# madmann91/bvh

Measured on AMD Instinct MI355X. Metric: Mrays/s closest-hit (1M-tri scene), higher is better.
Workload: dtype f32; 1 GPU; soup_1m: 1,000,000-triangle random soup (M3), worst-case incoherent; robust traversal, DefaultBuilder with thread pool (mini-trees) Quality::High built on the GPU (the reference's default configuration is thread pool + High); rays reordered for coherence inside the timed pass (library default for this tree size); tris=1000000, nodes=1866439, ray_batches=4, parallelism=single GPU, launched_by=single process

## Files before the change

bvh_amd/_lib.py:

```python
from __future__ import annotations

import ctypes as C
import os

HERE = os.path.dirname(os.path.abspath(__file__))
LIB_PATH = os.environ.get("BVH_AMD_LIB") or os.path.join(HERE, "lib", "libbvh_amd.so")

_lib = None


class BvhAmdError(RuntimeError):
    pass


class BuildConfig(C.Structure):
    _fields_ = [("quality", C.c_int), ("min_leaf_size", C.c_size_t), ("max_leaf_size", C.c_size_t),
                ("parallel_threshold", C.c_size_t)]


class Counters(C.Structure):
    _fields_ = [("node_pairs", C.c_ulonglong), ("prim_tests", C.c_ulonglong), ("leaves", C.c_ulonglong)]


class MiniTreeConfig(C.Structure):
# ... 37 lines not shown
    "bvh_amd_probe_record_walk": (_I, [_P, C.c_uint32, C.c_uint32, _I, _I, C.POINTER(C.c_float), C.POINTER(C.c_ulonglong), _P]),
    "bvh_amd_probe_mixed_walk": (_I, [_P, C.c_uint32, _P, C.c_uint32, C.c_uint32, _I, _I, _I, C.POINTER(C.c_float), C.POINTER(C.c_ulonglong), _P]),
    "bvh_amd_probe_record_walk_ex": (_I, [_P, C.c_uint32, C.c_uint32, _I, _I, _I, _I, C.POINTER(C.c_float), C.POINTER(C.c_ulonglong), _P]),
    "bvh_amd_release_cached_memory": (_I, []),
    "bvh_amd_cached_scratch_bytes": (_Z, []),
    "bvh_amd_scratch_cache_limit": (_Z, []),
    "bvh_amd_device_count": (_I, []),
    "bvh_amd_device_name": (_I, [_I, C.c_char_p, _Z]),
    "bvh_amd_device_select": (_I, [_I]),
    "bvh_amd_device_current": (_I, []),
    "bvh_amd_comm_unique_id": (_I, [_P]),
    "bvh_amd_comm_create": (_P, [_P, _I, _I]),
    "bvh_amd_comm_adopt": (_P, [_P]),
    "bvh_amd_comm_destroy": (None, [_P]),
    "bvh_amd_comm_rank": (_I, [_P]),
    "bvh_amd_comm_size": (_I, [_P]),
    "bvh_amd_comm_handle": (_P, [_P]),
    "bvh_amd_comm_broadcast": (_I, [_P, _P, _Z, _I, _P]),
    "bvh_amd_comm_cache_clear": (_I, []),
    "bvh_amd_rccl_library": (C.c_char_p, []),
    "bvh_thread_pool_create": (_P, [_Z]),
    "bvh_thread_pool_destroy": (None, [_P]),
    "bvh_amd_gather": (_I, [_P, _P, _Z, _Z, _P, _P]),
    "bvh_amd_pinhole_rays3f": (_I, [_P, _P, _P, _Z, _Z, _P, _P]),
    "bvh_amd_pinhole_rays3d": (_I, [_P, _P, _P, _Z, _Z, _P, _P]),
    "bvh_amd_shade_eyelight3f": (_I, [_P, _P, _P, _Z, _P, _P]),
    "bvh_amd_shade_eyelight3d": (_I, [_P, _P, _P, _Z, _P, _P]),
    "bvh_amd_device_alloc": (_P, [_Z]),
    "bvh_amd_device_free": (None, [_P]),
    "bvh_amd_copy_to_device": (_I, [_P, _P, _Z]),
    "bvh_amd_copy_to_host": (_I, [_P, _P, _Z]),
    "bvh_amd_synchronize": (_I, [_P]),
    "bvh_amd_std_sort_ids3f": (_I, [_P, _Z, _P, _P]),
    "bvh_amd_std_sort_ids3d": (_I, [_P, _Z, _P, _P]),
    "bvh_amd_radix_sort_pairs_u32": (_I, [_P, _P, _Z, _I, _P]),
}
_SIGS_T = {
    "bvh{S}_build": (_P, [_P, _P, _P, _Z, _P]),
    "bvh{S}_build_device": (_P, [_P, _P, _Z, _P, _I, _P]),
    "bvh{S}_build_sah": (_P, [_P, _P, _P, _Z, _P, _P]),
    "bvh{S}_build_device_sah": (_P, [_P, _P, _Z, _P, _I, _P, _P]),
    "bvh{S}_build_device_binned": (_P, [_P, _P, _Z, _P, _P, _Z, _P]),
    "bvh{S}_build_minitree_device": (_P, [_P, _P, _Z, _P, _P]),
    "bvh{S}_from_nodes": (_P, [_P, _Z, _P, _Z]),
    "bvh{S}_extract": (_P, [_P, _Z]),
    "bvh{S}_destroy": (None, [_P]),
    "bvh{S}_optimize": (None, [_P, _P]),
    "bvh{S}_optimize_config": (_I, [_P, _P]),
    "bvh{S}_refit": (None, [_P]),
    "bvh{S}_refit_status": (_I, [_P]),
    "bvh{S}_sync_device": (_I, [_P]),
    "bvh{S}_refit_boxes": (_I, [_P, _P, _Z, _P]),
    "bvh{S}_refit_tris": (_I, [_P, _P, _Z, _P, _P]),
    "bvh{S}_traversal_cost": (_I, [_P, C.POINTER(C.c_double), _P]),
    "bvh{S}_append_node": (None, [_P]),
    "bvh{S}_remove_last_node": (None, [_P]),
    "bvh_node{S}_set_prim_count": (None, [_P, _Z]),
    "bvh_node{S}_set_first_id": (None, [_P, _Z]),
    "bvh_node{S}_set_bbox": (None, [_P, _P]),
    "bvh{S}_save": (None, [_P, _P]),
    "bvh{S}_load": (_P, [_P]),
    "bvh{S}_serialize": (_Z, [_P, _P, _Z]),
    "bvh{S}_deserialize": (_P, [_P, _Z]),
    "bvh{S}_serialize_device": (_Z, [_P, _P, _Z, _P]),
    "bvh{S}_deserialize_device": (_P, [_P, _Z, _P]),
    "bvh{S}_broadcast": (_P, [_P, _I, _P, _P, _Z, C.POINTER(C.c_void_p), C.POINTER(C.c_size_t), _P]),
    "bvh{S}_replicate": (_I, [_P, _P, _Z, _I, C.POINTER(C.c_int), C.POINTER(C.c_void_p), C.POINTER(C.c_void_p)]),
    "bvh{S}_get_node": (_P, [_P, _Z]),
    "bvh{S}_get_prim_id": (_Z, [_P, _Z]),
    "bvh{S}_get_prim_count": (_Z, [_P]),
    "bvh{S}_get_node_count": (_Z, [_P]),
    "bvh_node{S}_is_leaf": (C.c_bool, [_P]),
    "bvh_node{S}_get_prim_count": (_Z, [_P]),
    "bvh_node{S}_get_first_id": (_Z, [_P]),
    "bvh{S}_copy_nodes": (None, [_P, _P]),
    "bvh{S}_copy_prim_ids": (None, [_P, _P]),
    "bvh{S}_device_prim_ids": (_P, [_P]),
    "bvh_amd_tri_bounds{S}": (_I, [_P, _Z, _P, _P, _P]),
    "bvh_amd_precompute_tris{S}": (_I, [_P, _P, _Z, _P, _P]),
    "bvh_amd_sphere_bounds{S}": (_I, [_P, _Z, _P, _P, _P]),
    "bvh{S}_intersect_rays_tri": (_I, [_P, _P, _P, _Z, _U, _P, _P, _P]),
    "bvh{S}_intersect_rays_sphere": (_I, [_P, _P, _P, _Z, _U, _P, _P, _P]),
    "bvh{S}_prepare_trace": (_I, [_P, _Z, _P]),
    "bvh{S}_closest_points_tri": (_I, [_P, _P, _P, _Z, _U, _P, _P, _P]),
    "bvh{S}_closest_points_sphere": (_I, [_P, _P, _P, _Z, _U, _P, _P, _P]),
    "bvh{S}_intersect_ray": (None, [_P, _P, _P]),
    "bvh{S}_intersect_ray_any": (None, [_P, _P, _P]),
    "bvh{S}_intersect_ray_robust": (None, [_P, _P, _P]),
    "bvh{S}_intersect_ray_any_robust": (None, [_P, _P, _P]),
    "bvh{S}_intersect_ray_visit": (_I, [_P, _P, _Z, _U, _P]),
}


class OptimizeProfile(C.Structure):
    _fields_ = [("iterations", C.c_uint), ("replayed", C.c_uint), ("replacements", C.c_ulonglong), ("heap_ms", C.c_float)]


class SahConfig(C.Structure):
    _fields_ = [("log_cluster_size", C.c_size_t), ("cost_ratio", C.c_double)]


class OptimizeConfig(C.Structure):
    _fields_ = [("batch_size_ratio", C.c_double), ("max_iter_count", C.c_size_t)]


def ray_visitor_types(suffix: str):
    scalar = C.c_float if suffix[1] == "f" else C.c_double
    leaf_t = C.CFUNCTYPE(C.c_bool, C.c_void_p, C.POINTER(scalar), C.c_size_t, C.c_size_t)
    inner_t = C.CFUNCTYPE(None, C.c_void_p, C.c_size_t)

    class Visitor(C.Structure):
        _fields_ = [("user_data", C.c_void_p), ("leaf_fn", leaf_t), ("inner_fn", inner_t)]
    return Visitor, leaf_t, inner_t


_ONLY_3D = ("bvh_amd_tri_bounds{S}", "bvh_amd_precompute_tris{S}", "bvh{S}_intersect_rays_tri", "bvh{S}_prepare_trace",
            "bvh{S}_build_minitree_device",
            "bvh{S}_closest_points_tri", "bvh{S}_closest_points_sphere",
            "bvh{S}_refit_tris", "bvh{S}_traversal_cost")


def exported_symbols():
    names = list(_SIGS)
    for s in ("3f", "3d", "2f", "2d"):
        names += [k.format(S=s) for k in _SIGS_T if s[0] == "3" or k not in _ONLY_3D]
        names += [f"bvh_node{s}_get_bbox"]
    return names


def load():
    global _lib
    if _lib is not None:
        return _lib
    import torch
    if not os.path.exists(LIB_PATH):
        raise BvhAmdError(f"{LIB_PATH} is missing: build it with `python -m bvh_amd.build` "
                          "(no fallback path exists)")
    lib = C.CDLL(LIB_PATH)
    for name, (res, args) in _SIGS.items():
        f = getattr(lib, name)
        f.restype, f.argtypes = res, args
    for s in ("3f", "3d", "2f", "2d"):
        for name, (res, args) in _SIGS_T.items():
            if s[0] == "2" and name in _ONLY_3D:
                continue
            f = getattr(lib, name.format(S=s))
            f.restype, f.argtypes = res, args
    lib.bvh_node3f_get_bbox.restype, lib.bvh_node3f_get_bbox.argtypes = BBox3f, [_P]
    lib.bvh_node3d_get_bbox.restype, lib.bvh_node3d_get_bbox.argtypes = BBox3d, [_P]
    lib.bvh_node2f_get_bbox.restype, lib.bvh_node2f_get_bbox.argtypes = BBox2f, [_P]
    lib.bvh_node2d_get_bbox.restype, lib.bvh_node2d_get_bbox.argtypes = BBox2d, [_P]
    _lib = lib
    return lib


def last_error() -> str:
    return load().bvh_amd_last_error().decode()


def check(rc: int, what: str):
    if rc != 0:
        raise BvhAmdError(f"{what} failed ({rc}): {last_error()}")
```

bvh_amd/api.py:

```python
from __future__ import annotations

import ctypes as C
import enum
from dataclasses import dataclass, field

import numpy as np

from . import _lib

INVALID = 0xFFFFFFFF
HITF = np.dtype([("prim", "<u4"), ("t", "<f4"), ("u", "<f4"), ("v", "<f4")])
HITD = np.dtype([("prim", "<u4"), ("pad", "<u4"), ("t", "<f8"), ("u", "<f8"), ("v", "<f8")])
NODEF = np.dtype([("bounds", "<f4", (6,)), ("index", "<u4")])
NODED = np.dtype([("bounds", "<f8", (6,)), ("index", "<u8")])
NODE2F = np.dtype([("bounds", "<f4", (4,)), ("index", "<u4")])
NODE2D = np.dtype([("bounds", "<f8", (4,)), ("index", "<u8")])
_NODE_DTYPES = {"3f": NODEF, "3d": NODED, "2f": NODE2F, "2d": NODE2D}


class Quality(enum.IntEnum):
    Low = 0
    Medium = 1
    High = 2

# ... 94 lines not shown
        return np.float32 if self._s[1] == "f" else np.float64

    @property
    def dim(self) -> int:
        return int(self._s[0])

    @property
    def node_count(self) -> int:
        return self._f("bvh{S}_get_node_count")(self._h)

    @property
    def prim_count(self) -> int:
        return self._f("bvh{S}_get_prim_count")(self._h)

    @property
    def nodes(self) -> np.ndarray:
        out = np.empty(self.node_count, dtype=_NODE_DTYPES[self._s])
        self._f("bvh{S}_copy_nodes")(self._h, out.ctypes.data_as(C.c_void_p))
        return out

    @property
    def prim_ids(self) -> np.ndarray:
        out = np.empty(self.prim_count, dtype=np.uint64)
        self._f("bvh{S}_copy_prim_ids")(self._h, out.ctypes.data_as(C.c_void_p))
        return out

    def device_prim_ids(self):
        torch = _torch()
        ptr = self._f("bvh{S}_device_prim_ids")(self._h)
        n = self.prim_count

        class _Holder:
            __cuda_array_interface__ = {"shape": (n,), "typestr": "<i4", "data": (ptr, False), "version": 2}
        t = torch.as_tensor(_Holder(), device="cuda")
        t._bvh_keepalive = self
        return t

    def optimize(self, thread_pool=None, batch_size_ratio=None, max_iter_count=None):
        _torch()
        if batch_size_ratio is not None or max_iter_count is not None:
            cfg = _lib.OptimizeConfig(0.05 if batch_size_ratio is None else float(batch_size_ratio),
                                      3 if max_iter_count is None else int(max_iter_count))
            _lib.check(self._f("bvh{S}_optimize_config")(self._h, C.byref(cfg)), "optimize")
            return
        _lib.check(self._f("bvh{S}_optimize_config")(self._h, None), "optimize")

    def refit(self):
        _torch()
        _lib.check(self._f("bvh{S}_refit_status")(self._h), "refit")

    def _prims_in(self, x, cols, what):
        torch = _torch()
        if not hasattr(x, "dtype"):
            x = np.asarray(x)
        dt = x.dtype
        want = torch.float32 if self._s[1] == "f" else torch.float64
        if dt not in (want, np.dtype(self.dtype), self.dtype):
            raise TypeError(f"{what}: the tree is {np.dtype(self.dtype).name}, the array is {dt}")
        return _dev(x, cols)

    def refit_boxes(self, bboxes):
        bb = self._prims_in(bboxes, 2 * self.dim, "refit_boxes")
        _lib.check(self._f("bvh{S}_refit_boxes")(self._h, bb.data_ptr(), bb.shape[0], _stream()), "refit_boxes")

    def refit_tris(self, tris9, out=None):
        torch = _torch()
        if self.dim != 3:
            raise TypeError("refit_tris: triangles are 3D (tri.h)")
        t = self._prims_in(tris9, 9, "refit_tris")
        if out is None:
            out = torch.empty((self.prim_count, 12), dtype=t.dtype, device=t.device)
        elif not (isinstance(out, torch.Tensor) and out.is_cuda and out.is_contiguous() and out.dtype == t.dtype and out.numel() == 12 * self.prim_count):
            raise TypeError("refit_tris: `out` must be a contiguous (prim_count, 12) device tensor of the tree's scalar type")
        _lib.check(self._f("bvh{S}_refit_tris")(self._h, t.data_ptr(), t.shape[0], out.data_ptr(), _stream()), "refit_tris")
        return out.reshape(-1, 12)

    def traversal_cost(self) -> float:
        _torch()
        if self.dim != 3:
            raise TypeError("traversal_cost: 3D trees only")
        cost = C.c_double(0.0)
        _lib.check(self._f("bvh{S}_traversal_cost")(self._h, C.byref(cost), _stream()), "traversal_cost")
        return float(cost.value)

    def set_node_bbox(self, node_id: int, lo, hi):
        node = self._f("bvh{S}_get_node")(self._h, node_id)
        ct = C.c_float if self._s[1] == "f" else C.c_double
        bb = (ct * (2 * self.dim))(*[float(v) for v in list(lo) + list(hi)])
        self._f("bvh_node{S}_set_bbox")(node, bb)

    def sync_device(self):
        _lib.check(self._f("bvh{S}_sync_device")(self._h), "sync_device")

    def sync_host(self):
        if not self._f("bvh{S}_get_node")(self._h, 0):
            raise _lib.BvhAmdError(_lib.last_error())

    def get_root(self):
        return self.nodes[0]

    def serialize(self) -> bytes:
        n = self._f("bvh{S}_serialize")(self._h, None, 0)
        buf = C.create_string_buffer(n)
        self._f("bvh{S}_serialize")(self._h, buf, n)
        return buf.raw

    @staticmethod
    def deserialize(data: bytes, dtype=np.float32, dim: int = 3) -> "Bvh":
        s = _suffix(np.dtype(dtype), dim)
        lib = _lib.load()
        _torch()
        return Bvh(getattr(lib, f"bvh{s}_deserialize")(data, len(data)), s)

    def serialize_device(self):
        torch = _torch()
        n = self._f("bvh{S}_serialize_device")(self._h, None, 0, _stream())
        buf = torch.empty(n, dtype=torch.uint8, device="cuda")
        if self._f("bvh{S}_serialize_device")(self._h, buf.data_ptr(), n, _stream()) != n:
            raise _lib.BvhAmdError(_lib.last_error())
        return buf

    @staticmethod
    def deserialize_device(buf, dtype=np.float32, dim: int = 3) -> "Bvh":
        torch = _torch()
        s = _suffix(np.dtype(dtype), dim)
        if not (buf.is_cuda and buf.dtype == torch.uint8 and buf.is_contiguous()):
            raise TypeError("deserialize_device takes a contiguous uint8 tensor resident on the GPU")
        return Bvh(getattr(_lib.load(), f"bvh{s}_deserialize_device")(buf.data_ptr(), buf.numel(), _stream()), s)

    def intersect_ray(self, ray, leaf_fn, any_hit: bool = False, robust: bool = False, inner_fn=None, start=None):
        lib = _lib.load()
        dt = np.float32 if self._s[1] == "f" else np.float64
        r = np.ascontiguousarray(ray, dtype=dt).reshape(2 * self.dim + 2)
        Visitor, leaf_t, inner_t = _lib.ray_visitor_types(self._s)
        failure = []

        def on_leaf(_user, t, begin, end):
            try:
                hit, new_t = leaf_fn(dt(t[0]), int(begin), int(end))
                t[0] = new_t
                return bool(hit)
            except BaseException as exc:
                failure.append(exc)
                t[0] = float("-inf")
                return True

        def on_inner(_user, first):
            try:
                if not failure:
                    inner_fn(int(first))
            except BaseException as exc:
                failure.append(exc)

        v = Visitor(None, leaf_t(on_leaf), inner_t(on_inner) if inner_fn is not None else inner_t())
        if start is None:
            start = (1 << 64) - 1
        rc = getattr(lib, f"bvh{self._s}_intersect_ray_visit")(self._h, r.ctypes.data, int(start), (RayFlags.ANY_HIT if any_hit else 0) | (RayFlags.ROBUST if robust else 0), C.byref(v))
        if failure:
            raise failure[0]
        _lib.check(rc, "intersect_ray_visit")

    def extract_bvh(self, root_id: int) -> "Bvh":
        h = getattr(_lib.load(), f"bvh{self._s}_extract")(self._h, int(root_id))
        return Bvh(h, self._s)

    @staticmethod
# ... 250 lines not shown
```

bvh_amd/csrc/capi.hip:

```cpp
#include "common.h"

#include <cstring>
#include <memory>

namespace bvh_amd {

template <typename T> int reinsertion_optimize_device(HostNode<T>* d_nodes, size_t node_count, hipStream_t stream, int dim);
template <typename T>
int reinsertion_optimize_config_device(HostNode<T>* d_nodes, size_t node_count, hipStream_t stream, int dim, double batch_size_ratio, size_t iterations);
void reinsertion_stats(unsigned out[2]);
void last_optimize_profile(bvh_amd_optimize_profile* out);
template <typename T>
int build_minitree_explicit(BvhImpl<T>& out, const T* d_bboxes, const T* d_centers, size_t n, const bvh_build_config& cfg, bool prune, T ratio,
                            bool optimize, uint32_t log2_grid, hipStream_t stream);
template <typename T>
int extract_device(BvhImpl<T>& out, const HostNode<T>* d_nodes, size_t node_count, const uint32_t* d_ids, size_t root_id, hipStream_t stream);
template <typename T> int refit_device(HostNode<T>* d_nodes, size_t node_count, hipStream_t stream);
template <typename T> int reachable_node_count(const HostNode<T>* d_nodes, size_t node_count, hipStream_t stream, size_t* out);
template <typename T> int relayout_on_device(BvhImpl<T>& b, const HostNode<T>* d_nodes, hipStream_t stream);

namespace {
thread_local std::string g_error;
}

// ... 221 lines not shown
    if (rc) return rc;
    rc = relayout_on_device<T>(b, b.d_nodes, nullptr);
    if (rc) return rc;
    HostNode<T> root;
    BVH_HIP_TRY(hipMemcpy(&root, b.d_nodes, sizeof(root), hipMemcpyDeviceToHost), BVH_AMD_ERR_HIP);
    b.root_index = static_cast<uint32_t>(root.index);
    for (int k = 0; k < 6; ++k) b.root_bounds[k] = root.bounds[k];
    if (b.host_valid) BVH_HIP_TRY(hipMemcpy(b.nodes.data(), b.d_nodes, bytes, hipMemcpyDeviceToHost), BVH_AMD_ERR_HIP);
    b.nodes2_valid = false;
    return BVH_AMD_OK;
}

template <typename T> BvhImpl<T>* extract(BvhImpl<T>* pb, size_t root_id) {
    if (!pb) { set_error("extract: null bvh"); return nullptr; }
    BvhImpl<T>& b = *pb;
    if (make_nodes_resident<T>(b)) return nullptr;
    if (!b.d_prim_ids) { set_error("extract: the BVH has no device prim ids"); return nullptr; }
    auto out = std::make_unique<BvhImpl<T>>();
    out->dim = b.dim;
    if (extract_device<T>(*out, b.d_nodes, b.node_count, b.d_prim_ids, root_id, nullptr)) return nullptr;
    return out.release();
}

template <typename T> int whole_array_is_one_tree(const HostNode<T>* d, size_t n) {
    size_t reachable = 0;
    const int rc = reachable_node_count<T>(d, n, nullptr, &reachable);
    if (rc) return rc;
    if (reachable != n)
        return fail(BVH_AMD_ERR_UNSUPPORTED, "optimize: " + std::to_string(n - reachable) + " of the " + std::to_string(n) +
                    " nodes are not reachable from the root (unused sibling pairs); extract_bvh(0) first, or remove them");
    return BVH_AMD_OK;
}
template <typename T> int optimize(BvhImpl<T>* b) {
    const int dim = b ? b->dim : 3;
    return on_resident_nodes<T>(b, [dim](HostNode<T>* d, size_t n) {
        const int rc = whole_array_is_one_tree<T>(d, n);
        return rc ? rc : reinsertion_optimize_device<T>(d, n, nullptr, dim);
    });
}
template <typename T> int optimize_config(BvhImpl<T>* b, const bvh_amd_optimize_config* config) {
    const int dim = b ? b->dim : 3;
    const bvh_amd_optimize_config c = config ? *config : bvh_amd_optimize_config{0.05, 3};
    return on_resident_nodes<T>(b, [dim, c](HostNode<T>* d, size_t n) {
        const int rc = whole_array_is_one_tree<T>(d, n);
        return rc ? rc : reinsertion_optimize_config_device<T>(d, n, nullptr, dim, c.batch_size_ratio, c.max_iter_count);
    });
}
template <typename T> int refit(BvhImpl<T>* b) {
    return on_resident_nodes<T>(b, [](HostNode<T>* d, size_t n) { return refit_device<T>(d, n, nullptr); });
}

template <typename T>
int refit_prims(BvhImpl<T>* pb, int src_kind, const T* d_src, size_t n_src, T* d_tris12_out, void* stream_, const char* who) {
    if (!pb) return fail(BVH_AMD_ERR_ARG, std::string(who) + ": null bvh");
    if (!d_src) return fail(BVH_AMD_ERR_ARG, std::string(who) + ": null primitive array");
    BvhImpl<T>& b = *pb;
    hipStream_t stream = static_cast<hipStream_t>(stream_);
    int cur = -1;
    BVH_HIP_TRY(hipGetDevice(&cur), BVH_AMD_ERR_HIP);
    if (cur != b.device) return fail(BVH_AMD_ERR_ARG, std::string(who) + ": BVH lives on another device than the current one");
    if (b.node_count == 0 || !b.d_prim_ids) return fail(BVH_AMD_ERR_ARG, std::string(who) + ": BVH has no device copy");
    if (b.max_prim_id < 0) {
        uint32_t largest = 0;
        const int rc = max_prim_id_device(b.d_prim_ids, b.prim_count, stream, &largest);
        if (rc) return rc;
        b.max_prim_id = largest;
    }
    if (b.prim_count && n_src <= static_cast<size_t>(b.max_prim_id))
        return fail(BVH_AMD_ERR_ARG, std::string(who) + ": " + std::to_string(n_src) + " primitives given, but prim_ids refers to primitive " +
                    std::to_string(b.max_prim_id) + " (the array is indexed by original primitive id)");
    const bool from_host = b.host_valid || !b.d_nodes || b.d_nodes_count != b.node_count;
    int rc = from_host ? b.wait_refit() : BVH_AMD_OK;
    if (rc) return rc;
    rc = make_nodes_resident<T>(b);
    if (rc) return rc;
    if (from_host || (b.pair_count && !b.d_pairs)) {
        const long long largest = b.max_prim_id;
        rc = relayout_on_device<T>(b, b.d_nodes, stream);
        if (rc) return rc;
        b.max_prim_id = largest;
    }
    rc = refit_prims_device<T>(b.d_nodes, b.d_pairs, b.node_count, src_kind, d_src, n_src, b.d_prim_ids, b.prim_count, stream);
    if (rc == BVH_AMD_OK && d_tris12_out) rc = launch_precompute_tris<T>(d_src, b.d_prim_ids, b.prim_count, d_tris12_out, stream);
    b.host_valid = false;
    b.nodes2_valid = false;
    const int rc2 = b.note_refit(stream);
    return rc ? rc : rc2;
}

template <typename T>
int traversal_cost_checked(const BvhImpl<T>* b, double* cost_out, void* stream) {
    if (!b || !cost_out) return fail(BVH_AMD_ERR_ARG, "traversal_cost: null bvh or output");
    int cur = -1;
    BVH_HIP_TRY(hipGetDevice(&cur), BVH_AMD_ERR_HIP);
    if (cur != b->device) return fail(BVH_AMD_ERR_ARG, "traversal_cost: BVH lives on another device than the current one");
    return traversal_cost<T>(*b, cost_out, static_cast<hipStream_t>(stream));
}

template <typename T> int sync_device(BvhImpl<T>* pb) {
    if (!pb) return fail(BVH_AMD_ERR_ARG, "sync_device: null bvh");
    BvhImpl<T>& b = *pb;
    int rc = b.dim == 2 ? b.sync_host2() : b.sync_host();
    if (rc) return rc;
    if (b.dim == 2) b.widen_host();
    if (b.d_nodes) { (void)hipFree(b.d_nodes); b.d_nodes = nullptr; }
    return upload_bvh<T>(b, nullptr);
}

template <typename T> struct CTypes2;
template <> struct CTypes2<float>  { using Bvh = bvh2f; using Node = bvh_node2f; using BBox = bvh_bbox2f; using Vec = bvh_vec2f; using Ray = bvh_ray2f; };
template <> struct CTypes2<double> { using Bvh = bvh2d; using Node = bvh_node2d; using BBox = bvh_bbox2d; using Vec = bvh_vec2d; using Ray = bvh_ray2d; };
template <typename T> BvhImpl<T>* impl2(typename CTypes2<T>::Bvh* b) { return reinterpret_cast<BvhImpl<T>*>(b); }
template <typename T> const BvhImpl<T>* impl2(const typename CTypes2<T>::Bvh* b) { return reinterpret_cast<const BvhImpl<T>*>(b); }
template <typename T> typename CTypes2<T>::Bvh* handle2(BvhImpl<T>* b) { return reinterpret_cast<typename CTypes2<T>::Bvh*>(b); }

template <typename T>
typename CTypes2<T>::Bvh* build2_device(const T* d_bb4, const T* d_cc2, size_t n, const bvh_build_config* config, bvh_amd_builder builder, void* stream) {
    if (!d_bb4 || !d_cc2 || n == 0) { set_error("build: empty input (the reference's behaviour is undefined for 0 primitives)"); return nullptr; }
    bvh_build_config cfg = config ? *config : default_config();
    if (cfg.min_leaf_size < 1 || cfg.min_leaf_size > cfg.max_leaf_size || cfg.max_leaf_size > 15) {
        set_error("build: need 1 <= min_leaf_size <= max_leaf_size <= 15 (4-bit primitive count, index.h:38)");
        return nullptr;
    }
    T *d_bb6 = nullptr, *d_cc3 = nullptr;
    BVH_HIP_TRY_PTR(hipMalloc(&d_bb6, n * 6 * sizeof(T)));
    hipError_t e = hipMalloc(&d_cc3, n * 3 * sizeof(T));
    auto b = std::make_unique<BvhImpl<T>>();
    b->dim = 2;
    int rc = e == hipSuccess ? launch_widen_inputs<T>(d_bb4, d_cc2, n, d_bb6, d_cc3, static_cast<hipStream_t>(stream))
                             : fail(BVH_AMD_ERR_HIP, std::string("build: ") + hipGetErrorString(e));
    if (rc == BVH_AMD_OK) rc = build_on_device<T>(*b, d_bb6, d_cc3, n, cfg, builder, static_cast<hipStream_t>(stream));
    (void)hipStreamSynchronize(static_cast<hipStream_t>(stream));
    (void)hipFree(d_bb6);
    if (d_cc3) (void)hipFree(d_cc3);
    return rc == BVH_AMD_OK ? handle2<T>(b.release()) : nullptr;
}

template <typename T>
typename CTypes2<T>::Bvh* build2_host(bvh_thread_pool* pool, const typename CTypes2<T>::BBox* bboxes, const typename CTypes2<T>::Vec* centers, size_t n,
                                      const bvh_build_config* config) {
    if (!bboxes || !centers || n == 0) { set_error("build: empty input"); return nullptr; }
    static_assert(sizeof(typename CTypes2<T>::BBox) == 4 * sizeof(T) && sizeof(typename CTypes2<T>::Vec) == 2 * sizeof(T));
    T *d_bb = nullptr, *d_cc = nullptr;
    BVH_HIP_TRY_PTR(hipMalloc(&d_bb, n * 4 * sizeof(T)));
    hipError_t e = hipMalloc(&d_cc, n * 2 * sizeof(T));
    if (e == hipSuccess) e = hipMemcpy(d_bb, bboxes, n * 4 * sizeof(T), hipMemcpyHostToDevice);
    if (e == hipSuccess) e = hipMemcpy(d_cc, centers, n * 2 * sizeof(T), hipMemcpyHostToDevice);
    typename CTypes2<T>::Bvh* out = nullptr;
    if (e == hipSuccess)
        out = build2_device<T>(d_bb, d_cc, n, config, pool ? BVH_AMD_BUILDER_DEFAULT_PARALLEL : BVH_AMD_BUILDER_DEFAULT_SERIAL, nullptr);
    else
        set_error(std::string("build: ") + hipGetErrorString(e));
    (void)hipDeviceSynchronize();
    (void)hipFree(d_bb);
    if (d_cc) (void)hipFree(d_cc);
    return out;
}

template <typename T>
BvhImpl<T>* adopt_nodes2(const HostNode2<T>* nodes, size_t nn, std::vector<size_t>&& ids) {
    auto b = std::make_unique<BvhImpl<T>>();
    b->dim = 2;
    b->nodes2.assign(nodes, nodes + nn);
    b->widen_host();
    b->prim_ids = std::move(ids);
    if (upload_bvh<T>(*b, nullptr) != BVH_AMD_OK) return nullptr;
// ... 234 lines not shown
        return build_minitree<T>(d_bb, d_cc, n, cfg, stream); }                                                     \
    bvh##S* bvh##S##_extract(bvh##S* b, size_t root_id) { return handle<T>(extract<T>(impl<T>(b), root_id)); }      \
    bvh##S* bvh##S##_from_nodes(const void* nodes, size_t nn, const size_t* ids, size_t np) {                       \
        return from_nodes<T>(nodes, nn, ids, np); }                                                                 \
    void bvh##S##_destroy(bvh##S* b) { delete impl<T>(b); }                                                         \
    void bvh##S##_optimize(bvh_thread_pool*, bvh##S* b) { loud_or_abort(optimize<T>(impl<T>(b)), "bvh" #S "_optimize"); } \
    int bvh##S##_optimize_config(bvh##S* b, const bvh_amd_optimize_config* c) { return optimize_config<T>(impl<T>(b), c); } \
    void bvh##S##_refit(bvh##S* b) { loud_or_abort(refit<T>(impl<T>(b)), "bvh" #S "_refit"); }                     \
    int bvh##S##_refit_status(bvh##S* b) { return refit<T>(impl<T>(b)); }                                           \
    int bvh##S##_sync_device(bvh##S* b) { return sync_device<T>(impl<T>(b)); }                                       \
    int bvh##S##_refit_boxes(bvh##S* b, const T* d_bb, size_t n, void* s) {                                         \
        return refit_prims<T>(impl<T>(b), REFIT_BOXES3, d_bb, n, nullptr, s, "refit_boxes"); }                       \
    int bvh##S##_refit_tris(bvh##S* b, const T* d_tris9, size_t n, T* d_tris12_out, void* s) {                      \
        return refit_prims<T>(impl<T>(b), REFIT_TRIS, d_tris9, n, d_tris12_out, s, "refit_tris"); }                  \
    int bvh##S##_traversal_cost(bvh##S* b, double* cost_out, void* s) { return traversal_cost_checked<T>(impl<T>(b), cost_out, s); } \
    void bvh##S##_append_node(bvh##S* b) {                                                                          \
        if (impl<T>(b)->sync_host() != BVH_AMD_OK) return;                                                           \
        impl<T>(b)->nodes.emplace_back(); impl<T>(b)->node_count = impl<T>(b)->nodes.size(); }                       \
    void bvh##S##_remove_last_node(bvh##S* b) {                                                                     \
        if (impl<T>(b)->sync_host() != BVH_AMD_OK || impl<T>(b)->nodes.empty()) return;                              \
        impl<T>(b)->nodes.pop_back(); impl<T>(b)->node_count = impl<T>(b)->nodes.size(); }                           \
    void bvh_node##S##_set_prim_count(bvh_node##S* n, size_t c) {                                                   \
        auto h = reinterpret_cast<HostNode<T>*>(n);                                                                 \
        h->index = (h->index & ~static_cast<IndexOf<T>::Type>(kCountMask)) | (static_cast<IndexOf<T>::Type>(c) & kCountMask); } \
    void bvh_node##S##_set_first_id(bvh_node##S* n, size_t f) {                                                     \
        auto h = reinterpret_cast<HostNode<T>*>(n);                                                                 \
        h->index = (static_cast<IndexOf<T>::Type>(f) << kCountBits) | (h->index & kCountMask); }                    \
    void bvh_node##S##_set_bbox(bvh_node##S* n, const bvh_bbox##S* bb) {                                            \
        auto h = reinterpret_cast<HostNode<T>*>(n);                                                                 \
        h->bounds[0] = bb->min.x; h->bounds[1] = bb->max.x; h->bounds[2] = bb->min.y; h->bounds[3] = bb->max.y;     \
        h->bounds[4] = bb->min.z; h->bounds[5] = bb->max.z; }                                                         \
    void bvh##S##_save(const bvh##S* b, FILE* f) { if (b && f) save<T>(*impl<T>(b), f); }                           \
    bvh##S* bvh##S##_load(FILE* f) { return f ? load<T>(f) : nullptr; }                                             \
    size_t bvh##S##_serialize(const bvh##S* b, void* out, size_t cap) { return b ? serialize<T>(*impl<T>(b), out, cap) : 0; } \
    bvh##S* bvh##S##_deserialize(const void* bytes, size_t size) { return deserialize<T>(bytes, size); }            \
    size_t bvh##S##_serialize_device(bvh##S* b, void* d_out, size_t cap, void* stream) { return serialize_device<T>(impl<T>(b), d_out, cap, stream); } \
    bvh##S* bvh##S##_deserialize_device(const void* d_bytes, size_t size, void* stream) {                           \
        return handle<T>(deserialize_from_device<T>(d_bytes, size, 3, static_cast<hipStream_t>(stream))); }         \
    bvh_node##S* bvh##S##_get_node(bvh##S* b, size_t i) {                                                          \
        if (impl<T>(b)->sync_host() != BVH_AMD_OK) return nullptr;                                                   \
        return reinterpret_cast<bvh_node##S*>(&impl<T>(b)->nodes[i]); }                                              \
    size_t bvh##S##_get_prim_id(const bvh##S* b, size_t i) {                                                        \
        if (impl<T>(b)->sync_host() != BVH_AMD_OK) return BVH_INVALID_PRIM_ID;                                       \
        return impl<T>(b)->prim_ids[i]; }                                                                            \
    size_t bvh##S##_get_prim_count(const bvh##S* b) { return impl<T>(b)->prim_count; }                              \
    size_t bvh##S##_get_node_count(const bvh##S* b) { return impl<T>(b)->node_count; }                              \
    bool bvh_node##S##_is_leaf(const bvh_node##S* n) { return (reinterpret_cast<const HostNode<T>*>(n)->index & kCountMask) != 0; } \
    size_t bvh_node##S##_get_prim_count(const bvh_node##S* n) { return reinterpret_cast<const HostNode<T>*>(n)->index & kCountMask; } \
    size_t bvh_node##S##_get_first_id(const bvh_node##S* n) { return reinterpret_cast<const HostNode<T>*>(n)->index >> kCountBits; } \
    bvh_bbox##S bvh_node##S##_get_bbox(const bvh_node##S* n) {                                                      \
        auto h = reinterpret_cast<const HostNode<T>*>(n);                                                           \
        bvh_bbox##S r; r.min.x = h->bounds[0]; r.max.x = h->bounds[1]; r.min.y = h->bounds[2]; r.max.y = h->bounds[3]; \
        r.min.z = h->bounds[4]; r.max.z = h->bounds[5]; return r; }                                                 \
    void bvh##S##_copy_nodes(const bvh##S* b, void* out) {                                                          \
        if (impl<T>(b)->sync_host() != BVH_AMD_OK) return;                                                           \
        std::memcpy(out, impl<T>(b)->nodes.data(), impl<T>(b)->nodes.size() * sizeof(HostNode<T>)); }               \
    void bvh##S##_copy_prim_ids(const bvh##S* b, size_t* out) {                                                     \
        if (impl<T>(b)->sync_host() != BVH_AMD_OK) return;                                                           \
        std::memcpy(out, impl<T>(b)->prim_ids.data(), impl<T>(b)->prim_ids.size() * sizeof(size_t)); }              \
    const uint32_t* bvh##S##_device_prim_ids(const bvh##S* b) { return impl<T>(b)->d_prim_ids; }                    \
    int bvh_amd_tri_bounds##S(const T* t, size_t n, T* bb, T* cc, void* s) {                                        \
        return launch_tri_bounds<T>(t, n, bb, cc, static_cast<hipStream_t>(s)); }                                   \
    int bvh_amd_precompute_tris##S(const T* t, const uint32_t* perm, size_t n, T* out, void* s) {                   \
        return launch_precompute_tris<T>(t, perm, n, out, static_cast<hipStream_t>(s)); }                           \
    int bvh_amd_sphere_bounds##S(const T* sp, size_t n, T* bb, T* cc, void* s) {                                    \
        return launch_sphere_bounds<T>(sp, n, bb, cc, static_cast<hipStream_t>(s)); }                               \
    int bvh##S##_intersect_rays_tri(const bvh##S* b, const T* prims, const bvh_ray##S* rays, size_t n, unsigned flags, \
                                    bvh_hit##S* hits, bvh_amd_counters* cnt, void* s) {                             \
        return intersect<T>(b, LEAF_TRIANGLE, prims, rays, n, flags, hits, cnt, s); }                               \
    int bvh##S##_intersect_rays_sphere(const bvh##S* b, const T* prims, const bvh_ray##S* rays, size_t n, unsigned flags, \
                                       bvh_hit##S* hits, bvh_amd_counters* cnt, void* s) {                          \
        return intersect<T>(b, LEAF_SPHERE, prims, rays, n, flags, hits, cnt, s); }                                 \
    int bvh##S##_closest_points_tri(const bvh##S* b, const T* prims, const T* queries, size_t n, unsigned flags,       \
                                    bvh_hit##S* hits, bvh_amd_counters* cnt, void* s) {                             \
        return closest<T>(b, LEAF_TRIANGLE, prims, queries, n, flags, hits, cnt, s); }                              \
    int bvh##S##_closest_points_sphere(const bvh##S* b, const T* prims, const T* queries, size_t n, unsigned flags,    \
                                       bvh_hit##S* hits, bvh_amd_counters* cnt, void* s) {                          \
        return closest<T>(b, LEAF_SPHERE, prims, queries, n, flags, hits, cnt, s); }                                \
    int bvh##S##_prepare_trace(const bvh##S* b, size_t n_rays_hint, void* s) {                                      \
        if (!b) return fail(BVH_AMD_ERR_ARG, "prepare_trace: null bvh");                                            \
        int cur = -1;                                                                                               \
        BVH_HIP_TRY(hipGetDevice(&cur), BVH_AMD_ERR_HIP);                                                           \
        if (cur != impl<T>(b)->device) return fail(BVH_AMD_ERR_ARG, "prepare_trace: BVH lives on another device than the current one"); \
        return prepare_trace<T>(*impl<T>(b), n_rays_hint, static_cast<hipStream_t>(s)); }

BVH_AMD_IMPL(float, 3f)
BVH_AMD_IMPL(double, 3d)

#define BVH_AMD_IMPL_RAY(T, S, CB, VIS, D, IMPL)                                                                         \
    void bvh##S##_intersect_ray(const bvh##S* b, const bvh_ray##S* r, const CB* cb) { intersect_ray_legacy<T, D>(IMPL<T>(b), r, cb, 0u); } \
    void bvh##S##_intersect_ray_any(const bvh##S* b, const bvh_ray##S* r, const CB* cb) {                           \
        intersect_ray_legacy<T, D>(IMPL<T>(b), r, cb, BVH_AMD_RAY_ANY_HIT); }                                        \
    void bvh##S##_intersect_ray_robust(const bvh##S* b, const bvh_ray##S* r, const CB* cb) {                        \
        intersect_ray_legacy<T, D>(IMPL<T>(b), r, cb, BVH_AMD_RAY_ROBUST); }                                         \
    void bvh##S##_intersect_ray_any_robust(const bvh##S* b, const bvh_ray##S* r, const CB* cb) {                    \
        intersect_ray_legacy<T, D>(IMPL<T>(b), r, cb, BVH_AMD_RAY_ANY_HIT | BVH_AMD_RAY_ROBUST); }                   \
    int bvh##S##_intersect_ray_visit(const bvh##S* b, const bvh_ray##S* r, size_t start, unsigned flags, const VIS* v) { \
        if (!v || !v->leaf_fn) return fail(BVH_AMD_ERR_ARG, "intersect_ray_visit: null visitor");                   \
        return intersect_ray_visit<T, D>(IMPL<T>(b), r, start, flags, v->leaf_fn, v->inner_fn, v->user_data); }

BVH_AMD_IMPL_RAY(float, 3f, bvh_intersect_callbackf, bvh_amd_ray_visitorf, 3, impl)
BVH_AMD_IMPL_RAY(double, 3d, bvh_intersect_callbackd, bvh_amd_ray_visitord, 3, impl)

#define BVH_AMD_IMPL2(T, S)                                                                                         \
    bvh##S* bvh##S##_build(bvh_thread_pool* pool, const bvh_bbox##S* bb, const bvh_vec##S* cc, size_t n,            \
                           const bvh_build_config* cfg) { return loud(build2_host<T>(pool, bb, cc, n, cfg), "bvh" #S "_build"); } \
    bvh##S* bvh##S##_build_device(const T* d_bb4, const T* d_cc2, size_t n, const bvh_build_config* cfg,            \
                                  enum bvh_amd_builder builder, void* stream) {                                     \
        return build2_device<T>(d_bb4, d_cc2, n, cfg, builder, stream); }                                           \
    bvh##S* bvh##S##_build_sah(bvh_thread_pool* pool, const bvh_bbox##S* bb, const bvh_vec##S* cc, size_t n,        \
                               const bvh_build_config* cfg, const bvh_amd_sah_config* sah) {                       \
        return with_sah(sah, [&] { return build2_host<T>(pool, bb, cc, n, cfg); }); }                               \
    bvh##S* bvh##S##_build_device_sah(const T* d_bb4, const T* d_cc2, size_t n, const bvh_build_config* cfg,        \
                                      enum bvh_amd_builder builder, const bvh_amd_sah_config* sah, void* stream) {  \
        return with_sah(sah, [&] { return build2_device<T>(d_bb4, d_cc2, n, cfg, builder, stream); }); }            \
    bvh##S* bvh##S##_build_device_binned(const T* d_bb4, const T* d_cc2, size_t n, const bvh_build_config* cfg,     \
                                         const bvh_amd_sah_config* sah, size_t bin_count, void* stream) {           \
        return with_bins(sah, bin_count, [&] { return build2_device<T>(d_bb4, d_cc2, n, cfg, BVH_AMD_BUILDER_BINNED, stream); }); } \
    bvh##S* bvh##S##_extract(bvh##S* b, size_t root_id) { return handle2<T>(extract<T>(impl2<T>(b), root_id)); }    \
    bvh##S* bvh##S##_from_nodes(const void* nodes, size_t nn, const size_t* ids, size_t np) {                       \
        return from_nodes2<T>(nodes, nn, ids, np); }                                                                \
    void bvh##S##_destroy(bvh##S* b) { delete impl2<T>(b); }                                                        \
    void bvh##S##_optimize(bvh_thread_pool*, bvh##S* b) { loud_or_abort(optimize<T>(impl2<T>(b)), "bvh" #S "_optimize"); } \
    int bvh##S##_optimize_config(bvh##S* b, const bvh_amd_optimize_config* c) { return optimize_config<T>(impl2<T>(b), c); } \
    void bvh##S##_refit(bvh##S* b) { loud_or_abort(refit<T>(impl2<T>(b)), "bvh" #S "_refit"); }                    \
    int bvh##S##_refit_status(bvh##S* b) { return refit<T>(impl2<T>(b)); }                                          \
    int bvh##S##_sync_device(bvh##S* b) { return sync_device<T>(impl2<T>(b)); }                                      \
    int bvh##S##_refit_boxes(bvh##S* b, const T* d_bb4, size_t n, void* s) {                                        \
        return refit_prims<T>(impl2<T>(b), REFIT_BOXES2, d_bb4, n, nullptr, s, "refit_boxes"); }                     \
    void bvh##S##_append_node(bvh##S* b) {                                                                          \
        if (impl2<T>(b)->sync_host2() != BVH_AMD_OK) return;                                                         \
        impl2<T>(b)->nodes2.emplace_back(); impl2<T>(b)->node_count = impl2<T>(b)->nodes2.size(); }                  \
    void bvh##S##_remove_last_node(bvh##S* b) {                                                                     \
        if (impl2<T>(b)->sync_host2() != BVH_AMD_OK || impl2<T>(b)->nodes2.empty()) return;                          \
        impl2<T>(b)->nodes2.pop_back(); impl2<T>(b)->node_count = impl2<T>(b)->nodes2.size(); }                      \
    void bvh_node##S##_set_prim_count(bvh_node##S* n, size_t c) {                                                   \
        auto h = reinterpret_cast<HostNode2<T>*>(n);                                                                \
        h->index = (h->index & ~static_cast<IndexOf<T>::Type>(kCountMask)) | (static_cast<IndexOf<T>::Type>(c) & kCountMask); } \
    void bvh_node##S##_set_first_id(bvh_node##S* n, size_t f) {                                                     \
        auto h = reinterpret_cast<HostNode2<T>*>(n);                                                                \
        h->index = (static_cast<IndexOf<T>::Type>(f) << kCountBits) | (h->index & kCountMask); }                    \
    void bvh_node##S##_set_bbox(bvh_node##S* n, const bvh_bbox##S* bb) {                                            \
        auto h = reinterpret_cast<HostNode2<T>*>(n);                                                                \
        h->bounds[0] = bb->min.x; h->bounds[1] = bb->max.x; h->bounds[2] = bb->min.y; h->bounds[3] = bb->max.y; }   \
    void bvh##S##_save(const bvh##S* b, FILE* f) {                                                                  \
        if (!b || !f) return;                                                                                        \
        std::vector<uint8_t> buf(stream_size2(*impl2<T>(b)));                                                        \
        serialize2(*impl2<T>(b), buf.data(), buf.size());                                                            \
        fwrite(buf.data(), 1, buf.size(), f); }                                                                      \
    bvh##S* bvh##S##_load(FILE* f) { return f ? load2<T>(f) : nullptr; }                                            \
    size_t bvh##S##_serialize(const bvh##S* b, void* out, size_t cap) { return b ? serialize2<T>(*impl2<T>(b), out, cap) : 0; } \
    bvh##S* bvh##S##_deserialize(const void* bytes, size_t size) { return deserialize2<T>(bytes, size); }           \
    size_t bvh##S##_serialize_device(bvh##S* b, void* d_out, size_t cap, void* stream) { return serialize_device<T>(impl2<T>(b), d_out, cap, stream); } \
    bvh##S* bvh##S##_deserialize_device(const void* d_bytes, size_t size, void* stream) {                           \
        return handle2<T>(deserialize_from_device<T>(d_bytes, size, 2, static_cast<hipStream_t>(stream))); }        \
    bvh_node##S* bvh##S##_get_node(bvh##S* b, size_t i) {                                                          \
        if (impl2<T>(b)->sync_host2() != BVH_AMD_OK) return nullptr;                                                 \
        return reinterpret_cast<bvh_node##S*>(&impl2<T>(b)->nodes2[i]); }                                            \
    size_t bvh##S##_get_prim_id(const bvh##S* b, size_t i) {                                                        \
        if (impl2<T>(b)->sync_host() != BVH_AMD_OK) return BVH_INVALID_PRIM_ID;                                      \
        return impl2<T>(b)->prim_ids[i]; }                                                                           \
    size_t bvh##S##_get_prim_count(const bvh##S* b) { return impl2<T>(b)->prim_count; }                             \
    size_t bvh##S##_get_node_count(const bvh##S* b) { return impl2<T>(b)->node_count; }                             \
    bool bvh_node##S##_is_leaf(const bvh_node##S* n) { return (reinterpret_cast<const HostNode2<T>*>(n)->index & kCountMask) != 0; } \
    size_t bvh_node##S##_get_prim_count(const bvh_node##S* n) { return reinterpret_cast<const HostNode2<T>*>(n)->index & kCountMask; } \
    size_t bvh_node##S##_get_first_id(const bvh_node##S* n) { return reinterpret_cast<const HostNode2<T>*>(n)->index >> kCountBits; } \
    bvh_bbox##S bvh_node##S##_get_bbox(const bvh_node##S* n) {                                                      \
// ... 56 lines not shown
```

bvh_amd/csrc/common.h:

```cpp
#pragma once

#include <hip/hip_runtime.h>

#include <cstddef>
#include <cstdint>
#include <cstring>
#include <string>
#include <atomic>
#include <mutex>
#include <vector>

#include "../../include/bvh_amd.h"

namespace bvh_amd {

constexpr unsigned kCountBits = 4;
constexpr uint32_t kCountMask = 15u;
constexpr int kWave = 64;

template <typename T> struct IndexOf;
template <> struct IndexOf<float>  { using Type = uint32_t; };
template <> struct IndexOf<double> { using Type = uint64_t; };

template <typename T>
// ... 1 lines not shown
    T bounds[6];
    typename IndexOf<T>::Type index;
};
static_assert(sizeof(HostNode<float>) == 28 && sizeof(HostNode<double>) == 56);

template <typename T>
struct HostNode2 {
    T bounds[4];
    typename IndexOf<T>::Type index;
};
static_assert(sizeof(HostNode2<float>) == 20 && sizeof(HostNode2<double>) == 40);

template <typename T> struct PairNode;
template <> struct alignas(64) PairNode<float> {
    float lb[6], rb[6];
    uint32_t li, ri;
    uint32_t pad[2];
};
template <> struct alignas(128) PairNode<double> {
    double lb[6], rb[6];
    uint32_t li, ri;
    uint32_t pad[6];
};
static_assert(sizeof(PairNode<float>) == 64 && sizeof(PairNode<double>) == 128);


template <typename T> struct HitOf;
template <> struct HitOf<float>  { using Type = bvh_hit3f; };
template <> struct HitOf<double> { using Type = bvh_hit3d; };

void set_error(const std::string& msg);
int fail(int code, const std::string& msg);
std::string current_error();

#define BVH_HIP_TRY(expr, code)                                                                     \
    do {                                                                                            \
        hipError_t e_ = (expr);                                                                     \
        if (e_ != hipSuccess)                                                                       \
            return ::bvh_amd::fail((code), std::string(#expr) + ": " + hipGetErrorString(e_));      \
    } while (0)

#define BVH_HIP_TRY_PTR(expr)                                                                       \
    do {                                                                                            \
        hipError_t e_ = (expr);                                                                     \
        if (e_ != hipSuccess) {                                                                     \
            ::bvh_amd::set_error(std::string(#expr) + ": " + hipGetErrorString(e_));                \
            return nullptr;                                                                         \
        }                                                                                           \
    } while (0)

enum : int { BVH_AMD_OK = 0, BVH_AMD_ERR_HIP = -1, BVH_AMD_ERR_ARG = -2, BVH_AMD_ERR_UNSUPPORTED = -3,
             BVH_AMD_ERR_OVERFLOW = -4 };

template <typename T>
struct BvhImpl {
    mutable std::vector<HostNode<T>> nodes;
    mutable std::vector<size_t> prim_ids;
    mutable std::atomic<bool> host_valid{true};
    mutable std::mutex host_mutex;
    size_t node_count = 0, prim_count = 0;
    int dim = 3;
    mutable std::vector<HostNode2<T>> nodes2;
    mutable std::atomic<bool> nodes2_valid{false};
    int sync_host2() const;
    void widen_host() const;
    HostNode<T>* d_nodes = nullptr;
    size_t d_nodes_count = 0;
    mutable T root_bounds[6] = {0, 0, 0, 0, 0, 0};
    int sync_host() const;
    HostNode<T>* h_root = nullptr;
    hipEvent_t refit_done = nullptr;
    mutable std::atomic<bool> root_pending{false};
    mutable std::mutex root_mutex;
    int wait_refit() const;
    int note_refit(hipStream_t stream);
    long long max_prim_id = -1;
    int device = -1;
    PairNode<T>* d_pairs = nullptr;
    size_t pair_count = 0;
    uint32_t* d_prim_ids = nullptr;
    uint32_t root_index = 0;
    mutable std::atomic<int> max_depth{-1};
    mutable std::atomic<float> expected_visits{0.0f};
    mutable std::atomic<uint32_t> launch_plan[2] = {};
    struct PlanSearch {
        int index = 0;
        static constexpr int kCandidates = 5;
        int trying = -1;
        uint8_t count[kCandidates] = {};
        uint8_t dropped = 0;
        bool pending = false;
        bool recorded = false;
        hipEvent_t start = nullptr, stop = nullptr;
        size_t rays = 0;
        float ns_per_ray[kCandidates] = {};
        size_t rays_of[kCandidates] = {};
    };
    mutable PlanSearch plan_search[2];
    mutable std::mutex plan_mutex;
    static constexpr uint32_t kWorkSlots = 64, kWorkStride = 4096;
    unsigned long long* d_work = nullptr;
    mutable std::atomic<uint32_t> work_next{0};
    mutable hipEvent_t work_done[kWorkSlots] = {};
    mutable bool work_busy[kWorkSlots] = {};
    mutable std::mutex work_mutex;
    ~BvhImpl();
};

#if defined(BVH_AMD_DEVELOPER)
inline int dev_env_int_(const char* name, int dflt) { const char* v = std::getenv(name); return v ? std::atoi(v) : dflt; }
inline bool dev_env_is_(const char* name, const char* value) { const char* v = std::getenv(name); return v && std::strcmp(v, value) == 0; }
#define BVH_DEV_INT(name, dflt) (::bvh_amd::dev_env_int_(name, dflt))
#define BVH_DEV_STR(name) (static_cast<const char*>(std::getenv(name)))
#define BVH_DEV_IS(name, value) (::bvh_amd::dev_env_is_(name, value))
#else
#define BVH_DEV_INT(name, dflt) (dflt)
#define BVH_DEV_STR(name) (static_cast<const char*>(nullptr))
#define BVH_DEV_IS(name, value) (false)
#endif

struct SahParams { uint32_t log_cluster = 0; double cost_ratio = 1.0; uint32_t bin_count = 8; };
SahParams& ambient_sah();
struct SahScope {
    SahParams saved;
    explicit SahScope(const SahParams& p) : saved(ambient_sah()) { ambient_sah() = p; }
    ~SahScope() { ambient_sah() = saved; }
    SahScope(const SahScope&) = delete;
    SahScope& operator=(const SahScope&) = delete;
};

hipStream_t& ambient_stream();
struct ScratchScope;
void scratch_forget(void* p);
struct StreamScope {
    hipStream_t saved;
    ScratchScope* scope;
    explicit StreamScope(hipStream_t s);
    ~StreamScope();
    StreamScope(const StreamScope&) = delete;
    StreamScope& operator=(const StreamScope&) = delete;
};
bool scratch_pool_enabled();
struct ScratchTag {
    size_t capacity = 0;
    bool pooled = false;
};
hipError_t scratch_alloc(void** p, size_t bytes, ScratchTag* tag);
void scratch_free(void* p, const ScratchTag& tag);
void scratch_cache_flush();
size_t scratch_cache_bytes();
size_t scratch_cache_limit();

int readback(void* dst, const void* d_src, size_t bytes, hipStream_t stream);

template <typename T> int upload_bvh(BvhImpl<T>& b, hipStream_t stream);
template <typename T> int tree_depth(const BvhImpl<T>& b, hipStream_t stream);
template <typename T> int prepare_trace(const BvhImpl<T>& b, size_t n_rays_hint, hipStream_t stream);

template <typename T> int relayout_on_device(BvhImpl<T>& b, const HostNode<T>* d_nodes, hipStream_t stream);

template <typename T> size_t wire_size(const BvhImpl<T>& b);
template <typename T> size_t serialize_to_device(const BvhImpl<T>& b, void* d_out, size_t cap, hipStream_t stream);
template <typename T> BvhImpl<T>* deserialize_from_device(const void* d_bytes, size_t size, int dim, hipStream_t stream);
template <typename T> int nodes_resident(BvhImpl<T>& b);
template <typename T> int validate_resident_nodes(const HostNode<T>* d_nodes, size_t nn, size_t np, hipStream_t stream, const char* who);

template <typename T>
int launch_traverse(const BvhImpl<T>& b, int leaf_kind, const T* d_prims, const T* d_rays, size_t n, unsigned flags,
                    typename HitOf<T>::Type* d_hits, bvh_amd_counters* d_counters, hipStream_t stream);
template <typename T>
int launch_closest(const BvhImpl<T>& b, int leaf_kind, const T* d_prims, const T* d_queries, size_t n, unsigned flags,
                   typename HitOf<T>::Type* d_hits, bvh_amd_counters* d_counters, hipStream_t stream);
void last_launch_plan(int out[4]);
int wave_times(unsigned long long* out, size_t capacity_waves, size_t* n_waves);
void last_plan_search(float ns_per_ray[5], int measurements[5], unsigned* dropped);
int set_experiment(const char* name, int value);
void set_tuning(int refill, int leaf, int coop, int parts);
const char* last_kernel_name();
bool last_launch_reordered();
void kernel_timing(bool on);
int kernel_times(float* ms_out, size_t capacity, size_t* count_out);
int reorder_times(float* ms_out, size_t capacity, size_t* count_out);
template <typename T>
int trace_ray_callbacks(const BvhImpl<T>& b, const T ray8[8], uint32_t start, bool any, bool robust,
                        bool (*leaf_fn)(void*, T*, size_t, size_t), void (*inner_fn)(void*, size_t), void* user);

template <typename T> int launch_tri_bounds(const T* d_tris9, size_t n, T* d_bb, T* d_cc, hipStream_t s);
template <typename T> int launch_precompute_tris(const T* d_tris9, const uint32_t* d_perm, size_t n, T* d_out, hipStream_t s);
template <typename T> int launch_sphere_bounds(const T* d_sph4, size_t n, T* d_bb, T* d_cc, hipStream_t s);
int launch_gather(const void* d_in, const uint32_t* d_perm, size_t n, size_t stride, void* d_out, hipStream_t s);
template <typename T> int launch_circle_bounds(const T* d_circles3, size_t n, T* d_bb4, T* d_cc2, hipStream_t s);
template <typename T> int launch_widen_inputs(const T* d_bb4, const T* d_cc2, size_t n, T* d_bb6, T* d_cc3, hipStream_t s);

template <typename T> int launch_pinhole_rays(const T eye[3], const T dir[3], const T up[3], size_t width, size_t height, T* d_rays, hipStream_t s);
template <typename T>
int launch_shade_eyelight(const T* d_tris12, const T* d_rays, const typename HitOf<T>::Type* d_hits, size_t n, uint8_t* d_rgb, hipStream_t s);

template <typename K>
int radix_sort_pairs(K* keys, uint32_t* vals, K* keys_tmp, uint32_t* vals_tmp, uint32_t n, uint32_t batch, int bits, hipStream_t stream,
                     uint32_t* hist_buf = nullptr, bool iota_vals = false, bool keys_wanted = true, uint32_t** vals_result = nullptr,
                     bool first_hist_done = false);
constexpr int kRadixTileU32 = 8192;
size_t radix_sort_hist_words(uint32_t n, uint32_t batch);
template <typename T>
int std_sort_ids(uint32_t* d_ids, const T* d_keys, uint32_t n, uint32_t batch, uint32_t astride, uint32_t istride, hipStream_t stream);

int exclusive_scan_u32(const uint32_t* in, uint32_t* out, uint32_t n, uint32_t* total_host, hipStream_t stream);

template <typename T>
int build_on_device(BvhImpl<T>& out, const T* d_bboxes, const T* d_centers, size_t n, const bvh_build_config& cfg,
                    bvh_amd_builder builder, hipStream_t stream);

enum { LEAF_TRIANGLE = 0, LEAF_SPHERE = 1 };

enum { REFIT_BOXES3 = 0, REFIT_BOXES2 = 1, REFIT_TRIS = 2 };
template <typename T>
int refit_prims_device(HostNode<T>* d_nodes, PairNode<T>* d_pairs, size_t node_count, int src_kind, const T* d_src, size_t n_src,
                       const uint32_t* d_prim_ids, size_t prim_count, hipStream_t stream);
int max_prim_id_device(const uint32_t* d_prim_ids, size_t prim_count, hipStream_t stream, uint32_t* out);
template <typename T> int traversal_cost(const BvhImpl<T>& b, double* cost_out, hipStream_t stream);

}
```

bvh_amd/csrc/trace_body.inc:

```
#ifndef BVH_TRACE_COOP
#define BVH_TRACE_COOP false
#endif
    constexpr int kDepth = kLdsDepth;
    constexpr int kSpill = 64 - kDepth;
    __shared__ uint32_t lds_stack[kDepth * kBlock];
    uint32_t spill[kSpill];
    const int tid = threadIdx.x;
    const int lane = tid & (kWave - 1);
    const uint64_t lanes_below = (uint64_t{1} << lane) - 1;

    bool have = false, done = false, drained = false, nan_ray = false;
    uint32_t part = a.parts > 1 ? blockIdx.x % a.parts : 0, parts_left = a.parts;
    unsigned long long ray_id = 0;
    T org[3], dir[3], inv[3], aux[3];
    T tmin = 0, tmax = 0;
    uint32_t oct[3] = {0, 0, 0};
    uint32_t top = 0, sp = 0;
    uint32_t hit_prim = BVH_AMD_INVALID;
    T hit_t = 0, hit_u = 0, hit_v = 0;
    unsigned long long n_pairs = 0, n_tests = 0, n_leaves = 0;
#if defined(BVH_AMD_DEVELOPER) && defined(__HIPCC__)
    unsigned long long wt_begin = 0, wt_last_refill = 0, wt_rays = 0, wt_refill_ticks = 0, wt_refills = 0;
    if (a.wave_times) wt_begin = __builtin_amdgcn_s_memrealtime();
#endif

    auto deep_slot = [&](uint32_t i) { return a.deep + (size_t{blockIdx.x} * kBlock + tid) * a.deep_cap + i; };
    auto push = [&](uint32_t v) {
        if (sp < kDepth) lds_stack[sp * kBlock + tid] = v;
        else if (!Deep) spill[min(sp - kDepth, static_cast<uint32_t>(kSpill - 1))] = v;
        else if (sp < kDepth + kSpill) spill[sp - kDepth] = v;
        else *deep_slot(min(sp - (kDepth + kSpill), a.deep_cap - 1)) = v;
        ++sp;
    };
    auto pop = [&]() -> uint32_t {
        --sp;
        uint32_t v = lds_word(&lds_stack[min(sp, static_cast<uint32_t>(kDepth - 1)) * kBlock + tid]);
        if (sp >= kDepth) {
            if (!Deep) v = spill[min(sp - kDepth, static_cast<uint32_t>(kSpill - 1))];
            else if (sp < kDepth + kSpill) v = spill[sp - kDepth];
            else v = *deep_slot(min(sp - (kDepth + kSpill), a.deep_cap - 1));
        }
        return v;
    };

    for (;;) {
        const uint64_t idle = __ballot(!have);
        const int n_idle = __popcll(idle);
        if (!drained && (n_idle >= a.refill_threshold || n_idle == kWave)) {
#if defined(BVH_AMD_DEVELOPER) && defined(__HIPCC__)
            unsigned long long wt_t0 = 0;
            if (a.wave_times) wt_t0 = __builtin_amdgcn_s_memrealtime();
#endif
            unsigned long long base = 0, part_end = a.n;
            if (a.one_shot) {
                base = (static_cast<unsigned long long>(blockIdx.x) * (kBlock / kWave) + (tid >> 6)) * kWave;
                drained = true;
            } else {
                if (lane == 0) base = atomicAdd(a.work + part * kTicketStride, static_cast<unsigned long long>(n_idle));
                base = __shfl(base, 0) + part * a.part_size;
                part_end = min(a.n, (part + 1ull) * a.part_size);
                if (base + n_idle >= part_end) {
                    part = part + 1 == a.parts ? 0 : part + 1;
                    if (--parts_left == 0) drained = true;
                } else if (a.stagger && part_end - (base + n_idle) < static_cast<unsigned long long>(a.stagger) * ((blockIdx.x * 8u) / gridDim.x)) {
                    drained = true;
                }
            }
            if (!have) {
                const unsigned long long ticket = base + __popcll(idle & lanes_below);
                if (ticket < part_end) {
                    const bool once = (a.stream_hints & 1u) != 0;
                    const unsigned long long my = a.order ? (once ? load_word_nt(a.order + ticket) : a.order[ticket]) : ticket;
                    T r[8];
                    if (D == 3) { if (once) load_ray_nt(a.rays + 8 * my, r); else load_ray(a.rays + 8 * my, r); }
                    else {
                        T q[6];
                        load_ray2(a.rays + 6 * my, q);
                        r[0] = q[0]; r[1] = q[1]; r[2] = T(0); r[3] = q[2]; r[4] = q[3]; r[5] = T(0); r[6] = q[4]; r[7] = q[5];
                    }
#pragma unroll
                    for (int k = 0; k < D; ++k) {
                        org[k] = r[k]; dir[k] = r[3 + k];
                        T d = dir[k];
                        T iv = Robust ? T(1) / d
                                      : (Num<T>::abs_(d) <= Num<T>::kEps ? Num<T>::copysign_(Num<T>::kMax, d) : T(1) / d);
                        inv[k] = iv;
                        aux[k] = Robust ? (Num<T>::finite(iv) ? Num<T>::bump2(iv) : iv) : (-iv) * org[k];
                        oct[k] = Num<T>::sign(d) ? 1u : 0u;
                    }
                    tmin = r[6]; tmax = r[7];
                    nan_ray = !(tmin == tmin) || !(tmax == tmax);
                    ray_id = my;
                    have = true; done = false;
                    sp = 0;
                    top = a.root_index;
                    hit_prim = BVH_AMD_INVALID; hit_t = tmax; hit_u = 0; hit_v = 0;
                }
            }
#if defined(BVH_AMD_DEVELOPER) && defined(__HIPCC__)
            if (a.wave_times) {
                asm volatile("s_waitcnt vmcnt(0)" ::: "memory");
                wt_last_refill = __builtin_amdgcn_s_memrealtime(); wt_rays += __popcll(__ballot(have)) - (kWave - n_idle);
                wt_refill_ticks += wt_last_refill - wt_t0; ++wt_refills;
            }
#endif
        }
        if (__ballot(have) == 0) {
            if (drained) break;
            continue;
        }

        for (;;) {
            const bool inner = have && !done && (top & kCountMask) == 0;
            const uint64_t inner_mask = __ballot(inner);
            if (!inner_mask) break;
            const int parked = __popcll(__ballot(have && !done && (top & kCountMask) != 0));
            if (parked >= a.leaf_threshold) break;
            T lb[6], rb[6];
            uint32_t li = 0, ri = 0;
            if constexpr (BVH_TRACE_COOP) coop_load_pair(a.pairs, a.pair_bytes, inner ? (top >> (kCountBits + 1)) : 0xFFFFFFFFu, lane, lb, rb, li, ri);
            if (inner) {
                if constexpr (!BVH_TRACE_COOP) load_pair(a.pairs + (top >> (kCountBits + 1)), lb, rb, li, ri);
                if (Stats) ++n_pairs;
                T l0 = tmin, l1 = tmax, r0 = tmin, r1 = tmax;
#pragma unroll
                for (int k = 0; k < D; ++k) {
                    const T ln = oct[k] ? lb[2 * k + 1] : lb[2 * k], lf = oct[k] ? lb[2 * k] : lb[2 * k + 1];
                    const T rn = oct[k] ? rb[2 * k + 1] : rb[2 * k], rf = oct[k] ? rb[2 * k] : rb[2 * k + 1];
                    T la, lz, ra, rz;
                    if (Robust) {
                        la = (ln - org[k]) * inv[k]; lz = (lf - org[k]) * aux[k];
                        ra = (rn - org[k]) * inv[k]; rz = (rf - org[k]) * aux[k];
                    } else {
                        la = Num<T>::fma_(ln, inv[k], aux[k]); lz = Num<T>::fma_(lf, inv[k], aux[k]);
                        ra = Num<T>::fma_(rn, inv[k], aux[k]); rz = Num<T>::fma_(rf, inv[k], aux[k]);
                    }
                    l0 = Num<T>::max_num(la, l0); l1 = Num<T>::min_num(lz, l1);
                    r0 = Num<T>::max_num(ra, r0); r1 = Num<T>::min_num(rz, r1);
                }
                const bool hl = !nan_ray && l0 <= l1, hr = !nan_ray && r0 <= r1;
                if (hl) {
                    uint32_t near_i = li;
                    if (hr) {
                        uint32_t far_i = ri;
                        if (!Any && l0 > r0) { near_i = ri; far_i = li; }
                        push(far_i);
                    }
                    top = near_i;
                } else if (hr) {
                    top = ri;
                } else if (sp == 0) {
                    done = true;
                } else {
                    top = pop();
                }
            }
        }

        if (have && !done && (top & kCountMask) != 0) {
            const uint32_t first = top >> kCountBits, count = top & kCountMask;
            if (Stats) ++n_leaves;
            for (uint32_t i = first; i < first + count; ++i) {
                if (Stats) ++n_tests;
                if (Leaf == LEAF_TRIANGLE) {
                    T p[12];
                    load_prim12(a.prims + static_cast<unsigned long long>(a.prim_stride) * i, p);
                    const T c0 = p[0] - org[0], c1 = p[1] - org[1], c2 = p[2] - org[2];
                    const T rx = dir[1] * c2 - dir[2] * c1, ry = dir[2] * c0 - dir[0] * c2, rz = dir[0] * c1 - dir[1] * c0;
                    const T inv_det = T(1) / dot3(p[9], p[10], p[11], dir[0], dir[1], dir[2]);
                    const T u = dot3(rx, ry, rz, p[6], p[7], p[8]) * inv_det;
                    const T v = dot3(rx, ry, rz, p[3], p[4], p[5]) * inv_det;
                    const T w = T(1) - u - v;
                    const T tol = -Num<T>::kEps;
                    if (u >= tol && v >= tol && w >= tol) {
                        const T t = dot3(p[9], p[10], p[11], c0, c1, c2) * inv_det;
                        if (t >= tmin && t <= tmax) { tmax = t; hit_t = t; hit_u = u; hit_v = v; hit_prim = i; }
                    }
                } else {
                    T qa, qb, qc;
                    if (D == 3) {
                        T s[4];
                        load_prim4(a.prims + 4ull * i, s);
                        const T o0 = org[0] - s[0], o1 = org[1] - s[1], o2 = org[2] - s[2];
                        qa = dot3(dir[0], dir[1], dir[2], dir[0], dir[1], dir[2]);
                        qb = T(2) * dot3(dir[0], dir[1], dir[2], o0, o1, o2);
                        qc = dot3(o0, o1, o2, o0, o1, o2) - s[3] * s[3];
                    } else {
                        const T* s = a.prims + 3ull * i;
                        const T o0 = org[0] - s[0], o1 = org[1] - s[1];
                        qa = dot2(dir[0], dir[1], dir[0], dir[1]);
                        qb = T(2) * dot2(dir[0], dir[1], o0, o1);
                        qc = dot2(o0, o1, o0, o1) - s[2] * s[2];
                    }
                    const T delta = qb * qb - T(4) * qa * qc;
                    if (delta >= 0) {
                        const T iv = -T(0.5) / qa;
                        const T root = Num<T>::sqrt_(delta);
                        const T t0 = pick_max((qb + root) * iv, tmin);
                        const T t1 = pick_min((qb - root) * iv, tmax);
                        if (t0 <= t1) { tmax = t0; hit_t = t0; hit_u = t1; hit_v = 0; hit_prim = i; }
                    }
                }
            }
            if (Any && hit_prim != BVH_AMD_INVALID) done = true;
            else if (sp == 0) done = true;
            else top = pop();
        }

        if (have && done) {
            if (a.stream_hints & 1u) store_hit_nt(a.hits + ray_id, hit_prim, hit_t, hit_u, hit_v);
            else store_hit(a.hits + ray_id, hit_prim, hit_t, hit_u, hit_v);
            have = false;
        }
    }

#if defined(BVH_AMD_DEVELOPER) && defined(__HIPCC__)
    if (a.wave_times && lane == 0) {
        uint32_t xcc = 0;
        asm volatile("s_getreg_b32 %0, hwreg(HW_REG_XCC_ID)" : "=s"(xcc));
        unsigned long long* w = a.wave_times + 6ull * (blockIdx.x * (kBlock / kWave) + (tid >> 6));
        w[0] = wt_begin; w[1] = wt_last_refill; w[2] = __builtin_amdgcn_s_memrealtime(); w[3] = (static_cast<unsigned long long>(xcc & 0xFu) << 32) | (wt_rays & 0xFFFFFFFFull);
        w[4] = wt_refill_ticks; w[5] = wt_refills;
    }
#endif
    if (Stats) {
#pragma unroll
        for (int off = 32; off > 0; off >>= 1) {
            n_pairs += __shfl_down(n_pairs, off);
            n_tests += __shfl_down(n_tests, off);
            n_leaves += __shfl_down(n_leaves, off);
        }
        if (lane == 0) {
            atomicAdd(&a.counters->node_pairs, n_pairs);
            atomicAdd(&a.counters->prim_tests, n_tests);
            atomicAdd(&a.counters->leaves, n_leaves);
        }
    }
```

bvh_amd/csrc/trace_device.h:

```cpp
#pragma once

#if defined(__HIPCC__)
#define BVH_AMD_KEEP_APART(v) asm volatile("" : "+v"(v))
#else
#define BVH_AMD_KEEP_APART(v) asm volatile("" : "+r"(v))
#endif

namespace bvh_amd {

namespace {

constexpr int kBlock = 256;
constexpr int kLdsDepth = 20;
constexpr int kRefillThreshold = 36;
constexpr int kRefillThresholdSmall = 20;
constexpr int kLeafThreshold = 12;
constexpr int kCoopRefillAny = 20, kCoopLeafAny = 20;
constexpr int kCoopRefillHeavy = 12, kCoopLeafHeavy = 12;


template <typename T> struct Num;
template <> struct Num<float> {
    static constexpr float kMax = 3.402823466e+38f, kEps = 1.1920928955078125e-07f;
    __device__ static bool finite(float x) { return (__float_as_uint(x) & 0x7F800000u) != 0x7F800000u; }
    __device__ static float bump2(float x) { return __uint_as_float(__float_as_uint(x) + 2u); }
    __device__ static bool sign(float x) { return (__float_as_uint(x) >> 31) != 0; }
    __device__ static float fma_(float a, float b, float c) { return __builtin_fmaf(a, b, c); }
    __device__ static float sqrt_(float x) { return __builtin_sqrtf(x); }
    __device__ static float abs_(float x) { return __builtin_fabsf(x); }
    __device__ static float copysign_(float a, float b) { return __builtin_copysignf(a, b); }
    __device__ static float max_num(float a, float b) { return __builtin_fmaxf(a, b); }
    __device__ static float min_num(float a, float b) { return __builtin_fminf(a, b); }
};
template <> struct Num<double> {
    static constexpr double kMax = 1.7976931348623157e+308, kEps = 2.220446049250313e-16;
    __device__ static bool finite(double x) {
        return (static_cast<uint32_t>(__double_as_longlong(x) >> 32) & 0x7FF00000u) != 0x7FF00000u;
    }
    __device__ static double bump2(double x) { return __longlong_as_double(__double_as_longlong(x) + 2ll); }
    __device__ static bool sign(double x) { return (__double_as_longlong(x) >> 63) != 0; }
    __device__ static double fma_(double a, double b, double c) { return __builtin_fma(a, b, c); }
    __device__ static double sqrt_(double x) { return __builtin_sqrt(x); }
    __device__ static double abs_(double x) { return __builtin_fabs(x); }
    __device__ static double copysign_(double a, double b) { return __builtin_copysign(a, b); }
    __device__ static double max_num(double a, double b) { return __builtin_fmax(a, b); }
    __device__ static double min_num(double a, double b) { return __builtin_fmin(a, b); }
};

template <typename T> __device__ inline T pick_min(T a, T b) { return a < b ? a : b; }
template <typename T> __device__ inline T pick_max(T a, T b) { return a > b ? a : b; }

template <typename T> __device__ inline T dot3(T a0, T a1, T a2, T b0, T b1, T b2) {
    return ((T(0) + a0 * b0) + a1 * b1) + a2 * b2;
}
__device__ inline uint32_t lds_word(const uint32_t* shared) {
#if defined(__HIP_DEVICE_COMPILE__)
    typedef __attribute__((address_space(3))) const volatile uint32_t LdsWord;
    return *(LdsWord*)shared;
#else
    return *shared;
#endif
}

template <typename T> __device__ inline T dot2(T a0, T a1, T b0, T b1) { return (T(0) + a0 * b0) + a1 * b1; }

constexpr uint32_t kTicketStride = 16;

template <typename T>
struct TraceArgs {
    const PairNode<T>* pairs;
    const T* prims;
    const T* rays;
    typename HitOf<T>::Type* hits;
    unsigned long long n;
    unsigned long long* work;
    unsigned long long part_size;
    uint32_t parts;
    bvh_amd_counters* counters;
    const uint32_t* order;
    uint32_t* deep;
    uint32_t deep_cap;
    uint32_t root_index;
    int refill_threshold;
    int leaf_threshold;
    uint32_t coop;
    uint32_t prim_stride;
    uint32_t stream_hints;
    uint32_t stagger;
    uint32_t one_shot;
    unsigned long long* wave_times;
    uint32_t pair_bytes = 0;
};

__device__ inline void load_pair(const PairNode<float>* p, float (&lb)[6], float (&rb)[6], uint32_t& li, uint32_t& ri) {
    const float4* q = reinterpret_cast<const float4*>(p);
    float4 a = q[0], b = q[1], c = q[2];
    uint2 d = reinterpret_cast<const uint2*>(p)[6];
    lb[0] = a.x; lb[1] = a.y; lb[2] = a.z; lb[3] = a.w; lb[4] = b.x; lb[5] = b.y;
    rb[0] = b.z; rb[1] = b.w; rb[2] = c.x; rb[3] = c.y; rb[4] = c.z; rb[5] = c.w;
    li = d.x; ri = d.y;
}
__device__ inline void load_pair(const PairNode<double>* p, double (&lb)[6], double (&rb)[6], uint32_t& li, uint32_t& ri) {
    const double2* q = reinterpret_cast<const double2*>(p);
#pragma unroll
    for (int i = 0; i < 3; ++i) { double2 v = q[i]; lb[2 * i] = v.x; lb[2 * i + 1] = v.y; }
#pragma unroll
    for (int i = 0; i < 3; ++i) { double2 v = q[3 + i]; rb[2 * i] = v.x; rb[2 * i + 1] = v.y; }
    uint2 d = reinterpret_cast<const uint2*>(p)[12];
    li = d.x; ri = d.y;
}

#if defined(__HIPCC__)
template <int CTRL> __device__ inline uint32_t quad_perm(uint32_t v) {
    return static_cast<uint32_t>(__builtin_amdgcn_mov_dpp(static_cast<int>(v), CTRL, 0xF, 0xF, true));
}
template <bool ByTwo> __device__ inline void quad_exchange4(uint32_t (&a)[4], uint32_t (&b)[4]) {
    const uint64_t lower = ByTwo ? 0x3333333333333333ull : 0x5555555555555555ull;
    uint32_t n0, n1, n2, n3;
    if (ByTwo)
        asm("s_nop 1\n\ts_mov_b64 vcc, %12\n\t"
            "v_cndmask_b32_dpp %0, %4, %8, vcc quad_perm:[2,3,0,1] row_mask:0xf bank_mask:0xf\n\t"
            "v_cndmask_b32_dpp %1, %5, %9, vcc quad_perm:[2,3,0,1] row_mask:0xf bank_mask:0xf\n\t"
            "v_cndmask_b32_dpp %2, %6, %10, vcc quad_perm:[2,3,0,1] row_mask:0xf bank_mask:0xf\n\t"
            "v_cndmask_b32_dpp %3, %7, %11, vcc quad_perm:[2,3,0,1] row_mask:0xf bank_mask:0xf\n\t"
            "s_not_b64 vcc, vcc\n\t"
            "v_cndmask_b32_dpp %4, %8, %4, vcc quad_perm:[2,3,0,1] row_mask:0xf bank_mask:0xf\n\t"
            "v_cndmask_b32_dpp %5, %9, %5, vcc quad_perm:[2,3,0,1] row_mask:0xf bank_mask:0xf\n\t"
            "v_cndmask_b32_dpp %6, %10, %6, vcc quad_perm:[2,3,0,1] row_mask:0xf bank_mask:0xf\n\t"
            "v_cndmask_b32_dpp %7, %11, %7, vcc quad_perm:[2,3,0,1] row_mask:0xf bank_mask:0xf"
            : "=&v"(n0), "=&v"(n1), "=&v"(n2), "=&v"(n3), "+v"(b[0]), "+v"(b[1]), "+v"(b[2]), "+v"(b[3])
            : "v"(a[0]), "v"(a[1]), "v"(a[2]), "v"(a[3]), "s"(lower) : "vcc", "scc");
    else
        asm("s_nop 1\n\ts_mov_b64 vcc, %12\n\t"
            "v_cndmask_b32_dpp %0, %4, %8, vcc quad_perm:[1,0,3,2] row_mask:0xf bank_mask:0xf\n\t"
            "v_cndmask_b32_dpp %1, %5, %9, vcc quad_perm:[1,0,3,2] row_mask:0xf bank_mask:0xf\n\t"
            "v_cndmask_b32_dpp %2, %6, %10, vcc quad_perm:[1,0,3,2] row_mask:0xf bank_mask:0xf\n\t"
            "v_cndmask_b32_dpp %3, %7, %11, vcc quad_perm:[1,0,3,2] row_mask:0xf bank_mask:0xf\n\t"
            "s_not_b64 vcc, vcc\n\t"
            "v_cndmask_b32_dpp %4, %8, %4, vcc quad_perm:[1,0,3,2] row_mask:0xf bank_mask:0xf\n\t"
            "v_cndmask_b32_dpp %5, %9, %5, vcc quad_perm:[1,0,3,2] row_mask:0xf bank_mask:0xf\n\t"
            "v_cndmask_b32_dpp %6, %10, %6, vcc quad_perm:[1,0,3,2] row_mask:0xf bank_mask:0xf\n\t"
            "v_cndmask_b32_dpp %7, %11, %7, vcc quad_perm:[1,0,3,2] row_mask:0xf bank_mask:0xf"
            : "=&v"(n0), "=&v"(n1), "=&v"(n2), "=&v"(n3), "+v"(b[0]), "+v"(b[1]), "+v"(b[2]), "+v"(b[3])
            : "v"(a[0]), "v"(a[1]), "v"(a[2]), "v"(a[3]), "s"(lower) : "vcc", "scc");
    a[0] = n0; a[1] = n1; a[2] = n2; a[3] = n3;
}
#elif defined(BVH_HOST_WAVE64)
template <int CTRL> inline uint32_t quad_perm(uint32_t v) {
    const int l = static_cast<int>(threadIdx.x) & 63;
    return wave_read(v, (l & ~3) | ((CTRL >> (2 * (l & 3))) & 3), true);
}
template <bool ByTwo> inline void quad_exchange4(uint32_t (&a)[4], uint32_t (&b)[4]) {
    const int l = static_cast<int>(threadIdx.x) & 63, bit = ByTwo ? 2 : 1, partner = l ^ bit;
    const bool lower = (l & bit) == 0;
    for (int i = 0; i < 4; ++i) {
        const uint32_t pa = wave_read(a[i], partner, true), pb = wave_read(b[i], partner, true);
        const uint32_t na = lower ? a[i] : pb, nb = lower ? pa : b[i];
        a[i] = na; b[i] = nb;
    }
}
#endif
constexpr uint32_t kNoRecordAt = 0xFFFFFFFFu << 6;
#if defined(__HIPCC__)
using PairRsrc = __amdgpu_buffer_rsrc_t;
__device__ inline PairRsrc pair_rsrc(const void* base, uint32_t bytes) {
    return __builtin_amdgcn_make_buffer_rsrc(const_cast<void*>(base), 0, static_cast<int>(bytes), 0x00020000);
}
__device__ inline uint4 load_chunk(PairRsrc r, uint32_t at) {
    const auto v = __builtin_amdgcn_raw_buffer_load_b128(r, static_cast<int>(at), 0, 0);
    return uint4{v[0], v[1], v[2], v[3]};
}
#elif defined(BVH_HOST_WAVE64)
struct PairRsrc { const char* base; };
inline PairRsrc pair_rsrc(const void* base, uint32_t) { return PairRsrc{static_cast<const char*>(base)}; }
inline uint4 load_chunk(PairRsrc r, uint32_t at) {
    if (at >= kNoRecordAt) return uint4{0, 0, 0, 0};
    return *reinterpret_cast<const uint4*>(r.base + at);
}
#endif
#if defined(__HIPCC__) || defined(BVH_HOST_WAVE64)
__device__ inline void coop_load_pair(const PairNode<float>* pairs, uint32_t pair_bytes, uint32_t want, int lane, float (&lb)[6], float (&rb)[6], uint32_t& li, uint32_t& ri) {
    const uint32_t at = want << 6, chunk = (static_cast<uint32_t>(lane) & 3u) * 16u;
    const PairRsrc r = pair_rsrc(pairs, pair_bytes);
    const uint4 c0 = load_chunk(r, quad_perm<0x00>(at) | chunk), c1 = load_chunk(r, quad_perm<0x55>(at) | chunk);
    const uint4 c2 = load_chunk(r, quad_perm<0xAA>(at) | chunk), c3 = load_chunk(r, quad_perm<0xFF>(at) | chunk);
    uint32_t v0[4] = {c0.x, c0.y, c0.z, c0.w}, v1[4] = {c1.x, c1.y, c1.z, c1.w}, v2[4] = {c2.x, c2.y, c2.z, c2.w}, v3[4] = {c3.x, c3.y, c3.z, c3.w};
    quad_exchange4<false>(v0, v1); quad_exchange4<false>(v2, v3);
    quad_exchange4<true>(v0, v2); quad_exchange4<true>(v1, v3);
    lb[0] = __uint_as_float(v0[0]); lb[1] = __uint_as_float(v0[1]); lb[2] = __uint_as_float(v0[2]); lb[3] = __uint_as_float(v0[3]);
    lb[4] = __uint_as_float(v1[0]); lb[5] = __uint_as_float(v1[1]); rb[0] = __uint_as_float(v1[2]); rb[1] = __uint_as_float(v1[3]);
    rb[2] = __uint_as_float(v2[0]); rb[3] = __uint_as_float(v2[1]); rb[4] = __uint_as_float(v2[2]); rb[5] = __uint_as_float(v2[3]);
    li = v3[0]; ri = v3[1];
}
__device__ inline void coop_load_pair(const PairNode<double>* pairs, uint32_t, uint32_t want, int lane, double (&lb)[6], double (&rb)[6], uint32_t& li, uint32_t& ri) {
    constexpr uint32_t kNone = 0xFFFFFFFFu;
    const uint32_t j = static_cast<uint32_t>(lane) & 3u;
    const uint32_t o0 = quad_perm<0x00>(want), o1 = quad_perm<0x55>(want), o2 = quad_perm<0xAA>(want), o3 = quad_perm<0xFF>(want);
    const char* base = reinterpret_cast<const char*>(pairs);
    const uint32_t chunk = j * 16u;
    uint4 c0 = {0, 0, 0, 0}, c1 = {0, 0, 0, 0}, c2 = {0, 0, 0, 0}, c3 = {0, 0, 0, 0}, d0 = {0, 0, 0, 0}, d1 = {0, 0, 0, 0}, d2 = {0, 0, 0, 0}, d3 = {0, 0, 0, 0};
    if (o0 != kNone) { c0 = *reinterpret_cast<const uint4*>(base + (o0 * 128u + chunk)); d0 = *reinterpret_cast<const uint4*>(base + (o0 * 128u + 64u + chunk)); }
    if (o1 != kNone) { c1 = *reinterpret_cast<const uint4*>(base + (o1 * 128u + chunk)); d1 = *reinterpret_cast<const uint4*>(base + (o1 * 128u + 64u + chunk)); }
    if (o2 != kNone) { c2 = *reinterpret_cast<const uint4*>(base + (o2 * 128u + chunk)); d2 = *reinterpret_cast<const uint4*>(base + (o2 * 128u + 64u + chunk)); }
    if (o3 != kNone) { c3 = *reinterpret_cast<const uint4*>(base + (o3 * 128u + chunk)); d3 = *reinterpret_cast<const uint4*>(base + (o3 * 128u + 64u + chunk)); }
    uint32_t v0[4] = {c0.x, c0.y, c0.z, c0.w}, v1[4] = {c1.x, c1.y, c1.z, c1.w}, v2[4] = {c2.x, c2.y, c2.z, c2.w}, v3[4] = {c3.x, c3.y, c3.z, c3.w};
    uint32_t w0[4] = {d0.x, d0.y, d0.z, d0.w}, w1[4] = {d1.x, d1.y, d1.z, d1.w}, w2[4] = {d2.x, d2.y, d2.z, d2.w}, w3[4] = {d3.x, d3.y, d3.z, d3.w};
    quad_exchange4<false>(v0, v1); quad_exchange4<false>(v2, v3);
    quad_exchange4<true>(v0, v2); quad_exchange4<true>(v1, v3);
    quad_exchange4<false>(w0, w1); quad_exchange4<false>(w2, w3);
    quad_exchange4<true>(w0, w2); quad_exchange4<true>(w1, w3);
    auto dbl = [](uint32_t lo, uint32_t hi) { return __longlong_as_double(static_cast<long long>((static_cast<unsigned long long>(hi) << 32) | lo)); };
    lb[0] = dbl(v0[0], v0[1]); lb[1] = dbl(v0[2], v0[3]); lb[2] = dbl(v1[0], v1[1]); lb[3] = dbl(v1[2], v1[3]);
    lb[4] = dbl(v2[0], v2[1]); lb[5] = dbl(v2[2], v2[3]); rb[0] = dbl(v3[0], v3[1]); rb[1] = dbl(v3[2], v3[3]);
    rb[2] = dbl(w0[0], w0[1]); rb[3] = dbl(w0[2], w0[3]); rb[4] = dbl(w1[0], w1[1]); rb[5] = dbl(w1[2], w1[3]);
    li = w2[0]; ri = w2[1];
    (void)w3;
}
#else
template <typename T> inline void coop_load_pair(const PairNode<T>* p, uint32_t, uint32_t want, int, T (&lb)[6], T (&rb)[6], uint32_t& li, uint32_t& ri) {
    if (want != 0xFFFFFFFFu) load_pair(p + want, lb, rb, li, ri);
}
#endif

__device__ inline void load_prim12(const float* p, float (&v)[12]) {
    const float4* q = reinterpret_cast<const float4*>(p);
    float4 a = q[0], b = q[1], c = q[2];
    v[0] = a.x; v[1] = a.y; v[2] = a.z; v[3] = a.w; v[4] = b.x; v[5] = b.y; v[6] = b.z; v[7] = b.w;
    v[8] = c.x; v[9] = c.y; v[10] = c.z; v[11] = c.w;
}
__device__ inline void load_prim12(const double* p, double (&v)[12]) {
    const double2* q = reinterpret_cast<const double2*>(p);
#pragma unroll
    for (int i = 0; i < 6; ++i) { double2 t = q[i]; v[2 * i] = t.x; v[2 * i + 1] = t.y; }
}
__device__ inline void load_prim4(const float* p, float (&v)[4]) {
    float4 a = *reinterpret_cast<const float4*>(p);
    v[0] = a.x; v[1] = a.y; v[2] = a.z; v[3] = a.w;
}
__device__ inline void load_prim4(const double* p, double (&v)[4]) {
    const double2* q = reinterpret_cast<const double2*>(p);
    double2 a = q[0], b = q[1];
    v[0] = a.x; v[1] = a.y; v[2] = b.x; v[3] = b.y;
}
__device__ inline void load_ray(const float* p, float (&v)[8]) {
    const float4* q = reinterpret_cast<const float4*>(p);
    float4 a = q[0], b = q[1];
    v[0] = a.x; v[1] = a.y; v[2] = a.z; v[3] = a.w; v[4] = b.x; v[5] = b.y; v[6] = b.z; v[7] = b.w;
}
__device__ inline void load_ray(const double* p, double (&v)[8]) {
    const double2* q = reinterpret_cast<const double2*>(p);
#pragma unroll
    for (int i = 0; i < 4; ++i) { double2 t = q[i]; v[2 * i] = t.x; v[2 * i + 1] = t.y; }
}
__device__ inline void load_ray_nt(const float* p, float (&v)[8]) {
#if defined(__HIP_DEVICE_COMPILE__)
    typedef float f4 __attribute__((ext_vector_type(4)));
    const f4* q = reinterpret_cast<const f4*>(p);
    const f4 a = __builtin_nontemporal_load(q), b = __builtin_nontemporal_load(q + 1);
    v[0] = a.x; v[1] = a.y; v[2] = a.z; v[3] = a.w; v[4] = b.x; v[5] = b.y; v[6] = b.z; v[7] = b.w;
#else
    load_ray(p, v);
#endif
}
__device__ inline void load_ray_nt(const double* p, double (&v)[8]) { load_ray(p, v); }
__device__ inline uint32_t load_word_nt(const uint32_t* p) {
#if defined(__HIP_DEVICE_COMPILE__)
    return __builtin_nontemporal_load(p);
#else
    return *p;
#endif
}
__device__ inline void load_ray2(const float* p, float (&v)[6]) {
    const float2* q = reinterpret_cast<const float2*>(p);
    float2 a = q[0], b = q[1], c = q[2];
    v[0] = a.x; v[1] = a.y; v[2] = b.x; v[3] = b.y; v[4] = c.x; v[5] = c.y;
}
__device__ inline void load_ray2(const double* p, double (&v)[6]) {
    const double2* q = reinterpret_cast<const double2*>(p);
#pragma unroll
    for (int i = 0; i < 3; ++i) { double2 t = q[i]; v[2 * i] = t.x; v[2 * i + 1] = t.y; }
}
__device__ inline void store_hit(bvh_hit3f* out, uint32_t prim, float t, float u, float v) {
    *reinterpret_cast<float4*>(out) = make_float4(__uint_as_float(prim), t, u, v);
}
__device__ inline void store_hit(bvh_hit3d* out, uint32_t prim, double t, double u, double v) {
    double2* q = reinterpret_cast<double2*>(out);
    q[0] = make_double2(__longlong_as_double(static_cast<long long>(prim)), t);
    q[1] = make_double2(u, v);
}
__device__ inline void store_hit_nt(bvh_hit3f* out, uint32_t prim, float t, float u, float v) {
#if defined(__HIP_DEVICE_COMPILE__)
    typedef float f4 __attribute__((ext_vector_type(4)));
    f4 h; h.x = __uint_as_float(prim); h.y = t; h.z = u; h.w = v;
    __builtin_nontemporal_store(h, reinterpret_cast<f4*>(out));
#else
    store_hit(out, prim, t, u, v);
#endif
}
__device__ inline void store_hit_nt(bvh_hit3d* out, uint32_t prim, double t, double u, double v) { store_hit(out, prim, t, u, v); }

}

}
```

bvh_amd/csrc/traverse.hip:

```cpp

#include "common.h"
#include "trace_device.h"
#include "ray_key.h"

#include <algorithm>
#include <chrono>
#include <cstdlib>
#include <cstring>
#include <memory>
#include <mutex>
#include <thread>
#include <type_traits>
#include <vector>

namespace bvh_amd {

namespace {

thread_local const char* g_last_kernel = "";
thread_local bool g_last_reordered = false;
thread_local int g_last_plan[4] = {0, 0, 0, 0};

struct KernelTimer {
    static constexpr size_t kRing = 256;
    bool on = false;
    size_t count = 0;
    std::pair<hipEvent_t, hipEvent_t> ring[kRing] = {};
    hipEvent_t begin[kRing] = {};
    bool begin_armed = false;
};
KernelTimer& kernel_timer() { static thread_local KernelTimer t; return t; }

template <typename T, bool Any, bool Robust, int Leaf, bool Stats, int D = 3, bool Deep = false>
__global__ void __launch_bounds__(kBlock) trace_kernel(TraceArgs<T> a) {
#include "trace_body.inc"
}

template <typename T, bool Any, bool Robust, int Leaf, bool Stats>
__global__ void __launch_bounds__(kBlock, 8) trace_kernel_coop(TraceArgs<T> a) {
    constexpr int D = 3;
    constexpr bool Deep = false;
#undef BVH_TRACE_COOP
#define BVH_TRACE_COOP true
#include "trace_body.inc"
#undef BVH_TRACE_COOP
}

template <typename T, bool Any, bool Robust, int Leaf, bool Stats, int D>
__global__ void __launch_bounds__(kBlock, sizeof(T) == 4 ? 8 : 4) trace_kernel_coop_nd(TraceArgs<T> a) {
    constexpr bool Deep = false;
#undef BVH_TRACE_COOP
#define BVH_TRACE_COOP true
#include "trace_body.inc"
#undef BVH_TRACE_COOP
}

template <typename T, bool Any, bool Robust, int Leaf>
__global__ void __launch_bounds__(kBlock) trace_kernel_plan_search(TraceArgs<T> a) {
    constexpr int D = 3;
    constexpr bool Deep = false, Stats = false;
#include "trace_body.inc"
}
template <typename T, bool Any, bool Robust, int Leaf>
__global__ void __launch_bounds__(kBlock, 8) trace_kernel_coop_plan_search(TraceArgs<T> a) {
    constexpr int D = 3;
    constexpr bool Deep = false, Stats = false;
#undef BVH_TRACE_COOP
#define BVH_TRACE_COOP true
#include "trace_body.inc"
#undef BVH_TRACE_COOP
}

#if defined(BVH_AMD_DEVELOPER)
__global__ void __launch_bounds__(256) k_check_order(const uint32_t* order, uint32_t n, uint32_t* bad) {
    const uint32_t i = blockIdx.x * 256 + threadIdx.x;
    if (i < n && order[i] >= n) {
        const uint32_t k = atomicAdd(&bad[0], 1u);
        if (k < 3) { bad[1 + 2 * k] = i; bad[2 + 2 * k] = order[i]; }
    }
}
#endif

template <typename T>
__global__ void __launch_bounds__(1024) ray_keys_kernel(const T* rays, uint32_t n, T lx, T ly, T lz, T sx, T sy, T sz, uint32_t* keys, uint32_t cells,
                                                        int hilbert_bits, int class_bits, T class_scale, uint32_t* hist, uint32_t tiles) {
    __shared__ uint32_t h[256];
    if (threadIdx.x < 256) h[threadIdx.x] = 0;
    __syncthreads();
    const uint32_t base = blockIdx.x * uint32_t(kRadixTileU32);
#pragma unroll
    for (int s0 = 0; s0 < kRadixTileU32 / 1024; ++s0) {
        const uint32_t i = base + uint32_t(s0) * 1024u + threadIdx.x;
        if (i < n) {
            T r[8];
            load_ray_nt(rays + 8ull * i, r);
            const uint32_t key = ray_key<T>(r, lx, ly, lz, sx, sy, sz, cells, hilbert_bits, class_bits, class_scale);
            keys[i] = key;
            atomicAdd(&h[key & 0xFFu], 1u);
        }
    }
    __syncthreads();
    if (threadIdx.x < 256) hist[size_t{threadIdx.x} * tiles + blockIdx.x] = h[threadIdx.x];
}

__global__ void __launch_bounds__(256) ray_entry_keys_kernel(const float* rays, uint32_t n, const PairNode<float>* pairs, uint32_t root_index, int depth,
                                                             uint32_t* keys) {
    const uint32_t i = blockIdx.x * 256 + threadIdx.x;
    if (i >= n) return;
    float r[8];
    load_ray(rays + 8ull * i, r);
    const float inv[3] = { 1.0f / r[3], 1.0f / r[4], 1.0f / r[5] };
    uint32_t cur = root_index, path = 0;
    int level = 0;
    for (; level < depth && (cur & kCountMask) == 0; ++level) {
        float lb[6], rb[6];
        uint32_t li, ri;
        load_pair(pairs + (cur >> (kCountBits + 1)), lb, rb, li, ri);
        float t0[2] = { r[6], r[6] }, t1[2] = { r[7], r[7] };
#pragma unroll
        for (int k = 0; k < 3; ++k) {
            const float a0 = (lb[2 * k] - r[k]) * inv[k], a1 = (lb[2 * k + 1] - r[k]) * inv[k];
            const float b0 = (rb[2 * k] - r[k]) * inv[k], b1 = (rb[2 * k + 1] - r[k]) * inv[k];
            t0[0] = fmaxf(t0[0], fminf(a0, a1)); t1[0] = fminf(t1[0], fmaxf(a0, a1));
            t0[1] = fmaxf(t0[1], fminf(b0, b1)); t1[1] = fminf(t1[1], fmaxf(b0, b1));
        }
        const bool hl = t0[0] <= t1[0], hr = t0[1] <= t1[1];
        if (!hl && !hr) break;
        const bool right = hl && hr ? t0[1] < t0[0] : hr;
        path = (path << 1) | (right ? 1u : 0u);
        cur = right ? ri : li;
    }
    path <<= (depth - level);
    const uint32_t oct = (Num<float>::sign(r[3]) ? 1u : 0u) | (Num<float>::sign(r[4]) ? 2u : 0u) | (Num<float>::sign(r[5]) ? 4u : 0u);
    keys[i] = (path << 3) | oct;
}

template <typename H>
__global__ void __launch_bounds__(256) original_ids_kernel(H* hits, size_t n, const uint32_t* prim_ids, uint32_t prim_count) {
    const size_t i = blockIdx.x * size_t{256} + threadIdx.x;
    if (i >= n) return;
    const uint32_t p = hits[i].prim;
    if (p < prim_count) hits[i].prim = prim_ids[p];
}

thread_local int t_refill = -1, t_leaf = -1, t_coop = -1, t_parts = -1;
struct Experiments { int grid_blocks = -1, stream_hints = -1, tri_stride = -1, key_curve = -1, key_bits = -1, step_events = -1, wave_times = -1, one_shot = -1,
                     key_class_bits = -1, key_class_scale = -1, stagger = -1; };
constexpr int kKeyClassBits = 0, kKeyClassScalePercent = 500;
constexpr uint32_t kStaggerHeavy = 100000, kStaggerLight = 50000, kStaggerDouble = 20000;
thread_local bool g_last_classes = false;
thread_local float g_search_ns[5] = {0, 0, 0, 0, 0};
thread_local int g_search_count[5] = {0, 0, 0, 0, 0};
thread_local unsigned g_search_dropped = 0;
thread_local Experiments t_exp;
#if defined(BVH_AMD_DEVELOPER)
constexpr size_t kWaveTimeWords = 6, kWaveTimeWaves = 8 * 256 * (kBlock / kWave) * 2;
thread_local unsigned long long* t_wave_times = nullptr;
thread_local size_t t_wave_times_waves = 0;
#endif
thread_local std::pair<hipEvent_t, hipEvent_t>* t_calibration = nullptr;

int coop_fetch_forced() {
    static const int knob = BVH_DEV_INT("BVH_AMD_COOP", -1);
    return t_coop >= 0 ? (t_coop != 0) : knob < 0 ? -1 : (knob != 0);
}

struct Grid { int blocks = 0; };

template <typename K>
int persistent_grid(K kernel, int device, Grid& g) {
    int per_cu = 0, cus = 0;
    BVH_HIP_TRY(hipOccupancyMaxActiveBlocksPerMultiprocessor(&per_cu, kernel, kBlock, 0), BVH_AMD_ERR_HIP);
    BVH_HIP_TRY(hipDeviceGetAttribute(&cus, hipDeviceAttributeMultiprocessorCount, device), BVH_AMD_ERR_HIP);
    if (per_cu < 1) per_cu = 1;
    if (per_cu > 8) per_cu = 8;
    g.blocks = per_cu * cus;
    return BVH_AMD_OK;
}

template <typename T, bool Any, bool Robust, int Leaf, bool Stats, int D, bool Deep, bool Coop = false>
int launch_variant_d(const BvhImpl<T>& b, const TraceArgs<T>& args, hipStream_t stream, const char* name) {
    static thread_local int cached_blocks[16] = {0};
    void (*kernel)(TraceArgs<T>) = nullptr;
    constexpr bool CoopNd = Coop && !(std::is_same_v<T, float> && D == 3);
    if constexpr (CoopNd) kernel = trace_kernel_coop_nd<T, Any, Robust, Leaf, Stats, D>;
    else if constexpr (Coop) kernel = trace_kernel_coop<T, Any, Robust, Leaf, Stats>;
    else kernel = trace_kernel<T, Any, Robust, Leaf, Stats, D, Deep>;
    if constexpr (std::is_same_v<T, float> && D == 3 && !Deep && !Stats) {
        if (t_calibration) {
            if constexpr (Coop) kernel = trace_kernel_coop_plan_search<T, Any, Robust, Leaf>;
            else kernel = trace_kernel_plan_search<T, Any, Robust, Leaf>;
        }
    }
    int& blocks = cached_blocks[b.device & 15];
    if (blocks == 0) {
        Grid g;
        int rc = persistent_grid(kernel, b.device, g);
        if (rc) return rc;
        blocks = g.blocks;
    }
    unsigned long long need = (args.n + kBlock - 1) / kBlock;
    int grid = static_cast<int>(need < static_cast<unsigned long long>(blocks) ? need : blocks);
    if (args.one_shot) grid = static_cast<int>(need);
    else if constexpr (!Coop && std::is_same_v<T, float>) {
        int cus = blocks / 7 > 0 ? blocks / 7 : 1;
        (void)hipDeviceGetAttribute(&cus, hipDeviceAttributeMultiprocessorCount, b.device);
        const int cap = 6 * cus;
        if (grid > cap) grid = cap;
    }
    static const int grid_env = BVH_DEV_INT("BVH_AMD_GRID_BLOCKS", 0);
    if (!args.one_shot) {
        if (grid_env > 0 && grid > grid_env) grid = grid_env;
        if (t_exp.grid_blocks > 0 && grid > t_exp.grid_blocks) grid = t_exp.grid_blocks;
    }
    if (grid < 1) grid = 1;
    (void)name;
    static const std::string head = std::string(CoopNd ? "trace_kernel_coop_nd<" : Coop ? "trace_kernel_coop<" : "trace_kernel<") + (std::is_same_v<T, float> ? "float" : "double") + ", " +
                                    (Any ? "true" : "false") + ", " + (Robust ? "true" : "false") + ", " + std::to_string(Leaf) + ", " + (Stats ? "true" : "false");
    static const std::string symbol = CoopNd ? head + ", " + std::to_string(D) + ">" : Coop ? head + ">" : head + ", " + std::to_string(D) + ", " + (Deep ? "true" : "false") + ">";
    g_last_kernel = symbol.c_str();
    KernelTimer& timer = kernel_timer();
    hipEvent_t stop = nullptr;
    if (timer.on) {
        std::pair<hipEvent_t, hipEvent_t>& ev = timer.ring[timer.count % KernelTimer::kRing];
        if (!timer.begin_armed && timer.begin[timer.count % KernelTimer::kRing]) {
            (void)hipEventDestroy(timer.begin[timer.count % KernelTimer::kRing]);
            timer.begin[timer.count % KernelTimer::kRing] = nullptr;
        }
        timer.begin_armed = false;
        if (!ev.first) {
// ... 148 lines not shown
                }
            }
            if (!stop && !dead && (n_events == a.max_events || snap_used + sp > a.snap_words)) stop = true;
            if (stop) {
                if (!error) { if (sp >= a.stack_cap) error = 1; else put(sp++, top); }
                break;
            }
            if (dead) continue;
            events[3 * n_events] = top; events[3 * n_events + 1] = snap_used; events[3 * n_events + 2] = sp;
            for (uint32_t i = 0; i < sp; ++i) snaps[snap_used + i] = get(i);
            snap_used += sp;
            ++n_events;
        }
        a.out[0] = n_events; a.out[1] = finished; a.out[2] = error;
        __hip_atomic_store(&a.out[3], a.seq, __ATOMIC_RELEASE, __HIP_MEMORY_SCOPE_SYSTEM);
        s_sp = sp;
    }
    __syncthreads();
    sp = s_sp;
    for (uint32_t i = lane; i < sp && i < kStepLds; i += kWave) a.scratch[1 + i] = s_stack[i];
    if (lane == 0) a.scratch[0] = sp;
}

struct StepContext {
    int device = -1;
    hipStream_t stream = nullptr;
    uint32_t* pinned = nullptr;
    uint32_t* scratch = nullptr;
    uint32_t stack_cap = 0, snap_words = 0;
    uint32_t seq = 0;
    void release() {
        if (stream) (void)hipStreamSynchronize(stream);
        if (pinned) (void)hipHostFree(pinned);
        if (scratch) (void)hipFree(scratch);
        if (stream) (void)hipStreamDestroy(stream);
        pinned = nullptr; scratch = nullptr; stream = nullptr; stack_cap = 0; device = -1;
    }
    ~StepContext() { release(); }
    int ensure(int dev, uint32_t cap) {
        if (device == dev && stack_cap >= cap) return BVH_AMD_OK;
        release();
        BVH_HIP_TRY(hipStreamCreateWithFlags(&stream, hipStreamNonBlocking), BVH_AMD_ERR_HIP);
        snap_words = std::max<uint32_t>(16384u, 4 * cap);
        const size_t words = size_t{1} + cap + kStepHeader + 3 * size_t{kStepEvents} + snap_words;
        BVH_HIP_TRY(hipHostMalloc(reinterpret_cast<void**>(&pinned), words * sizeof(uint32_t), hipHostMallocCoherent), BVH_AMD_ERR_HIP);
        std::memset(pinned, 0, words * sizeof(uint32_t));
        BVH_HIP_TRY(hipMalloc(reinterpret_cast<void**>(&scratch), (size_t{1} + cap) * sizeof(uint32_t)), BVH_AMD_ERR_HIP);
        device = dev; stack_cap = cap;
        return BVH_AMD_OK;
    }
};
struct StepContextPool {
    std::vector<std::unique_ptr<StepContext>> contexts;
    size_t depth = 0;
};
thread_local StepContextPool t_steps;
struct StepContextClaim {
    StepContext* ctx;
    StepContextClaim() {
        if (t_steps.depth == t_steps.contexts.size()) t_steps.contexts.push_back(std::make_unique<StepContext>());
        ctx = t_steps.contexts[t_steps.depth++].get();
    }
    ~StepContextClaim() { --t_steps.depth; }
    StepContextClaim(const StepContextClaim&) = delete;
    StepContextClaim& operator=(const StepContextClaim&) = delete;
};

}

void last_launch_plan(int out[4]) { for (int k = 0; k < 4; ++k) out[k] = g_last_plan[k]; }
void set_tuning(int refill, int leaf, int coop, int parts) { t_refill = refill; t_leaf = leaf; t_coop = coop; t_parts = parts; }
int set_experiment(const char* name, int value) {
    const std::string k = name ? name : "";
    if (k == "grid_blocks") t_exp.grid_blocks = value;
    else if (k == "stream_hints") t_exp.stream_hints = value;
    else if (k == "tri_stride") t_exp.tri_stride = value;
    else if (k == "key_curve") t_exp.key_curve = value;
    else if (k == "key_bits") t_exp.key_bits = value;
    else if (k == "step_events") t_exp.step_events = value;
    else if (k == "one_shot") t_exp.one_shot = value;
    else if (k == "stagger") t_exp.stagger = value;
    else if (k == "key_class_bits") t_exp.key_class_bits = value;
    else if (k == "key_class_scale") t_exp.key_class_scale = value;
    else if (k == "wave_times") {
#if defined(BVH_AMD_DEVELOPER)
        t_exp.wave_times = value;
#else
        return fail(BVH_AMD_ERR_ARG, "bvh_amd_experiment: 'wave_times' exists in the developer library only (python -m bvh_amd.build --developer)");
#endif
    }
    else if (k == "reset") t_exp = Experiments{};
    else return fail(BVH_AMD_ERR_ARG, "bvh_amd_experiment: unknown knob '" + k + "'");
    return BVH_AMD_OK;
}
int wave_times(unsigned long long* out, size_t capacity_waves, size_t* n_waves) {
#if defined(BVH_AMD_DEVELOPER)
    if (n_waves) *n_waves = t_wave_times_waves;
    if (!out || !t_wave_times) return BVH_AMD_OK;
    BVH_HIP_TRY(hipDeviceSynchronize(), BVH_AMD_ERR_HIP);
    BVH_HIP_TRY(hipMemcpy(out, t_wave_times, std::min(capacity_waves, t_wave_times_waves) * kWaveTimeWords * sizeof(unsigned long long), hipMemcpyDeviceToHost), BVH_AMD_ERR_HIP);
    return BVH_AMD_OK;
#else
    (void)out; (void)capacity_waves;
    if (n_waves) *n_waves = 0;
    return fail(BVH_AMD_ERR_ARG, "bvh_amd_wave_times: developer library only");
#endif
}
void last_plan_search(float ns_per_ray[5], int measurements[5], unsigned* dropped) {
    for (int c = 0; c < 5; ++c) { if (ns_per_ray) ns_per_ray[c] = g_search_ns[c]; if (measurements) measurements[c] = g_search_count[c]; }
    if (dropped) *dropped = g_search_dropped;
}
const char* last_kernel_name() { return g_last_kernel; }
bool last_launch_reordered() { return g_last_reordered; }

void kernel_timing(bool on) {
    KernelTimer& t = kernel_timer();
    t.on = on;
    t.count = 0;
}

int kernel_times(float* ms_out, size_t capacity, size_t* count_out) {
    KernelTimer& t = kernel_timer();
    const size_t have = std::min<size_t>(t.count, KernelTimer::kRing), n = std::min(have, capacity);
    for (size_t i = 0; i < n; ++i) {
        const std::pair<hipEvent_t, hipEvent_t>& ev = t.ring[(t.count - n + i) % KernelTimer::kRing];
        BVH_HIP_TRY(hipEventSynchronize(ev.second), BVH_AMD_ERR_HIP);
        BVH_HIP_TRY(hipEventElapsedTime(&ms_out[i], ev.first, ev.second), BVH_AMD_ERR_HIP);
    }
    if (count_out) *count_out = n;
    return BVH_AMD_OK;
}

int reorder_times(float* ms_out, size_t capacity, size_t* count_out) {
    KernelTimer& t = kernel_timer();
    const size_t have = std::min<size_t>(t.count, KernelTimer::kRing), n = std::min(have, capacity);
    for (size_t i = 0; i < n; ++i) {
        const size_t k = (t.count - n + i) % KernelTimer::kRing;
        ms_out[i] = 0.0f;
        if (!t.begin[k]) continue;
        BVH_HIP_TRY(hipEventSynchronize(t.ring[k].first), BVH_AMD_ERR_HIP);
        BVH_HIP_TRY(hipEventElapsedTime(&ms_out[i], t.begin[k], t.ring[k].first), BVH_AMD_ERR_HIP);
    }
    if (count_out) *count_out = n;
    return BVH_AMD_OK;
}

template <typename T>
static int to_original_ids(const BvhImpl<T>& b, typename HitOf<T>::Type* d_hits, size_t n, hipStream_t stream) {
    if (!b.d_prim_ids) return fail(BVH_AMD_ERR_ARG, "intersect_rays: BVH has no device prim ids");
    hipLaunchKernelGGL(original_ids_kernel<typename HitOf<T>::Type>, dim3(static_cast<unsigned>((n + 255) / 256)), dim3(256), 0, stream, d_hits, n,
                       b.d_prim_ids, static_cast<uint32_t>(b.prim_count));
    BVH_HIP_TRY(hipGetLastError(), BVH_AMD_ERR_HIP);
    return BVH_AMD_OK;
}

constexpr float kReorderMinVisits = 100.0f;

struct Plan { bool reorder; bool coop; int refill, leaf; bool classes = false; };

template <typename T>
static int launch_planned(const BvhImpl<T>& b, int leaf_kind, const T* d_prims, const T* d_rays, size_t n, unsigned flags,
                          typename HitOf<T>::Type* d_hits, bvh_amd_counters* d_counters, hipStream_t stream, const Plan* plan)
{
    if (n == 0) return BVH_AMD_OK;
    if (!d_prims || !d_rays || !d_hits) return fail(BVH_AMD_ERR_ARG, "intersect_rays: null device pointer");
    if (b.node_count == 0 || !b.d_work) return fail(BVH_AMD_ERR_ARG, "intersect_rays: BVH has no device copy");
// ... 7 lines not shown
            bool found = false;
            for (uint32_t i = 0; i < BvhImpl<T>::kWorkSlots && !found; ++i) {
                const uint32_t s = (from + i) % BvhImpl<T>::kWorkSlots;
                if (!b.work_busy[s]) { slot = s; found = true; }
            }
            if (found) break;
            lock.unlock();
            std::this_thread::yield();
            lock.lock();
        }
        if (!b.work_done[slot]) BVH_HIP_TRY(hipEventCreateWithFlags(&b.work_done[slot], hipEventDisableTiming), BVH_AMD_ERR_HIP);
        else BVH_HIP_TRY(hipStreamWaitEvent(stream, b.work_done[slot], 0), BVH_AMD_ERR_HIP);
        b.work_busy[slot] = true;
        b.work_next.store((slot + 1) % BvhImpl<T>::kWorkSlots);
        slot_event = b.work_done[slot];
    }
    unsigned long long* work = b.d_work + size_t{slot} * BvhImpl<T>::kWorkStride;
    if (KernelTimer& timer = kernel_timer(); timer.on) {
        hipEvent_t& ev = timer.begin[timer.count % KernelTimer::kRing];
        if (!ev) (void)hipEventCreate(&ev);
        if (ev) timer.begin_armed = hipEventRecord(ev, stream) == hipSuccess;
    }
    TraceArgs<T> args{};
    args.pairs = b.d_pairs; args.prims = d_prims; args.rays = d_rays; args.hits = d_hits;
    args.pair_bytes = static_cast<uint32_t>(std::min<size_t>(b.pair_count * sizeof(PairNode<T>), 0xFFFFFFFFu));
    args.n = n; args.work = work; args.counters = d_counters; args.root_index = b.root_index;
    args.order = nullptr;
    args.prim_stride = leaf_kind == LEAF_TRIANGLE ? (t_exp.tri_stride > 0 ? static_cast<uint32_t>(t_exp.tri_stride) : 12u) : 4u;
    args.stream_hints = 0;
    args.one_shot = (t_exp.one_shot >= 0 ? t_exp.one_shot > 0 : n <= (size_t{1} << 18)) && !d_counters ? 1u : 0u;
    static const int parts_env = BVH_DEV_INT("BVH_AMD_PARTS", 0);
    args.parts = t_parts > 0 ? std::min(t_parts, 256) : parts_env > 0 ? std::min(parts_env, 256) : n < 65536 ? 1 : 8;
    args.part_size = ((n + args.parts - 1) / args.parts + 63) / 64 * 64;
    args.deep = nullptr; args.deep_cap = 0;
    StreamScope scope(stream);
    void* deep_mem = nullptr;
    void* sort_mem = nullptr;
    ScratchTag deep_tag, sort_tag;
    auto release = [&](int rc) {
        (void)hipEventRecord(slot_event, stream);
        { std::lock_guard<std::mutex> lock(b.work_mutex); b.work_busy[slot] = false; }
        if (deep_mem) scratch_free(deep_mem, deep_tag);
        if (sort_mem) scratch_free(sort_mem, sort_tag);
        return rc;
    };
    if (d_counters) {
        const hipError_t e = hipMemsetAsync(d_counters, 0, sizeof(bvh_amd_counters), stream);
        if (e != hipSuccess) return release(fail(BVH_AMD_ERR_HIP, std::string("intersect_rays: hipMemsetAsync: ") + hipGetErrorString(e)));
    }
    {
        int rc = tree_depth<T>(b, stream);
        if (rc) return release(rc);
        const int max_depth = b.max_depth.load();
        if (max_depth > 64) {
            int cus = 0;
            if (hipDeviceGetAttribute(&cus, hipDeviceAttributeMultiprocessorCount, b.device) != hipSuccess) return release(fail(BVH_AMD_ERR_HIP, "intersect_rays: hipDeviceGetAttribute"));
            const size_t lanes = size_t{8} * cus * kBlock;
            const size_t cap = static_cast<size_t>(max_depth - 64 + 1);
            if (lanes * cap > (size_t{1} << 32))
                return release(fail(BVH_AMD_ERR_UNSUPPORTED, "intersect_rays: the tree is too deep for the traversal stack (" + std::to_string(max_depth) + " levels)"));
            const hipError_t e = scratch_alloc(&deep_mem, lanes * cap * sizeof(uint32_t), &deep_tag);
            if (e != hipSuccess) { deep_mem = nullptr; return release(fail(BVH_AMD_ERR_HIP, std::string("intersect_rays: stack spill buffer: ") + hipGetErrorString(e))); }
            args.deep = static_cast<uint32_t*>(deep_mem); args.deep_cap = static_cast<uint32_t>(cap);
            args.one_shot = 0;
        }
    }
    static const int refill_env = BVH_DEV_INT("BVH_AMD_REFILL", 0);
    static const int leaf_env = BVH_DEV_INT("BVH_AMD_LEAF", 0);
    const bool beyond_l2 = b.pair_count * sizeof(PairNode<T>) > (size_t{32} << 20);
    const bool heavy = beyond_l2 && b.expected_visits.load() >= kReorderMinVisits;
    const bool any_hit = (flags & BVH_AMD_RAY_ANY_HIT) != 0;
    const int forced = coop_fetch_forced();
    const bool coop_capable = true;
    if (plan) {
        args.coop = coop_capable && plan->coop ? 1u : 0u;
        args.refill_threshold = plan->refill; args.leaf_threshold = plan->leaf;
    } else {
        args.coop = (coop_capable && (forced >= 0 ? forced != 0 : (any_hit || (heavy && n >= (size_t{1} << 21))))) ? 1u : 0u;
        const int refill_lane = n <= (size_t{1} << 21) && std::is_same_v<T, float> ? kRefillThresholdSmall : kRefillThreshold;
        const int refill_default = !args.coop ? refill_lane : any_hit ? kCoopRefillAny : heavy ? kCoopRefillHeavy : kCoopRefillAny;
        const int leaf_default = !args.coop ? kLeafThreshold : any_hit ? kCoopLeafAny : heavy ? kCoopLeafHeavy : kCoopLeafAny;
        args.refill_threshold = t_refill > 0 ? t_refill : refill_env > 0 ? refill_env : refill_default;
        args.leaf_threshold = t_leaf > 0 ? t_leaf : leaf_env > 0 ? leaf_env : leaf_default;
    }
    auto zero_tickets = [&]() -> int {
        const hipError_t e = hipMemsetAsync(work, 0, size_t{args.parts} * kTicketStride * sizeof(unsigned long long), stream);
        return e == hipSuccess ? BVH_AMD_OK : fail(BVH_AMD_ERR_HIP, std::string("intersect_rays: hipMemsetAsync: ") + hipGetErrorString(e));
    };
    if (b.dim == 2) {
        if (leaf_kind != LEAF_SPHERE) return release(fail(BVH_AMD_ERR_ARG, "intersect_rays: a 2D BVH traces circles (Sphere<T, 2>) only"));
        if (const int rc0 = zero_tickets()) return release(rc0);
        int rc2 = dispatch<T, LEAF_SPHERE, 2>(b, args, flags, d_counters != nullptr, stream);
        if (rc2 == BVH_AMD_OK && (flags & BVH_AMD_RAY_ORIGINAL_IDS)) rc2 = to_original_ids<T>(b, d_hits, n, stream);
        return release(rc2);
    }
    const bool reorder = (flags & BVH_AMD_RAY_SORTED) ? n > 4096
                       : (flags & BVH_AMD_RAY_UNSORTED) ? false
                       : plan ? plan->reorder && n > 4096
                       : n >= (size_t{1} << 20) && beyond_l2 && b.expected_visits.load() >= kReorderMinVisits;
    g_last_reordered = reorder && n < (size_t{1} << 31);
    args.stream_hints = t_exp.stream_hints >= 0 ? static_cast<uint32_t>(t_exp.stream_hints) : g_last_reordered ? 1u : 0u;
    args.parts = t_parts > 0 ? std::min(t_parts, 256) : parts_env > 0 ? std::min(parts_env, 256) : n < 65536 ? 1 : g_last_reordered ? 8 : 32;
    args.part_size = ((n + args.parts - 1) / args.parts + 63) / 64 * 64;
    if (const int rc0 = zero_tickets()) return release(rc0);
    if (g_last_reordered) {
        const uint32_t n32 = static_cast<uint32_t>(n);
        const size_t words = 4 * n + radix_sort_hist_words(n32, 1);
        hipError_t e = scratch_alloc(&sort_mem, words * sizeof(uint32_t), &sort_tag);
        if (e != hipSuccess) {
            sort_mem = nullptr;
            (void)hipGetLastError();
            if (flags & BVH_AMD_RAY_SORTED) return release(fail(BVH_AMD_ERR_HIP, std::string("intersect_rays: no scratch for BVH_AMD_RAY_SORTED: ") + hipGetErrorString(e)));
            g_last_reordered = false;
        }
    }
    if (g_last_reordered) {
        const uint32_t n32 = static_cast<uint32_t>(n);
        uint32_t *keys = static_cast<uint32_t*>(sort_mem), *vals = keys + n, *kt = vals + n, *vt = kt + n, *hist = vt + n;
        T lo[3], sc[3];
        if (const int rc0 = b.wait_refit()) return release(rc0);
        for (int k = 0; k < 3; ++k) {
            const T ext = b.root_bounds[2 * k + 1] - b.root_bounds[2 * k];
            lo[k] = b.root_bounds[2 * k];
            sc[k] = ext > T(0) ? T(64) / ext : T(0);
        }
        static const int entry_depth = std::min(29, BVH_DEV_INT("BVH_AMD_RAY_KEY_DEPTH", 0));
        int key_bits = 21;
        bool entry_keys = false, first_hist_done = false;
        if constexpr (std::is_same_v<T, float>) entry_keys = entry_depth > 0 && b.dim == 3;
        if constexpr (std::is_same_v<T, float>) {
            if (entry_keys) {
                hipLaunchKernelGGL(ray_entry_keys_kernel, dim3((n32 + 255) / 256), dim3(256), 0, stream, d_rays, n32, args.pairs, args.root_index, entry_depth, keys);
                key_bits = entry_depth + 3;
            }
        }
        if (!entry_keys) {
            static const int cell_bits_env = std::max(1, std::min(8, BVH_DEV_INT("BVH_AMD_RAY_KEY_BITS", 7)));
            const int cell_bits = t_exp.key_bits > 0 ? std::min(8, t_exp.key_bits) : cell_bits_env;
            const T rescale = static_cast<T>(1u << cell_bits) / T(64);
            const int class_bits = cell_bits < 3 ? 0 : t_exp.key_class_bits >= 0 ? std::min(3, t_exp.key_class_bits) : (plan && plan->classes) ? 1 : kKeyClassBits;
            g_last_classes = class_bits > 0;
            const T class_scale = static_cast<T>(t_exp.key_class_scale > 0 ? t_exp.key_class_scale : kKeyClassScalePercent) / T(100);
            const uint32_t tiles = (n32 + kRadixTileU32 - 1) / kRadixTileU32;
            hipLaunchKernelGGL(ray_keys_kernel<T>, dim3(tiles), dim3(1024), 0, stream, d_rays, n32, lo[0], lo[1], lo[2], sc[0] * rescale, sc[1] * rescale,
                               sc[2] * rescale, keys, 1u << cell_bits, t_exp.key_curve == 0 ? 0 : cell_bits,
                               class_bits, class_scale, hist, tiles);
            first_hist_done = true;
            key_bits = 3 * cell_bits + 3;
        }
        uint32_t* order = nullptr;
        int rc = radix_sort_pairs<uint32_t>(keys, vals, kt, vt, n32, 1, key_bits, stream, hist, true, false, &order, first_hist_done);
        if (rc) return release(rc);
        args.order = order;
#if defined(BVH_AMD_DEVELOPER)
        if (getenv("BVH_AMD_CHECK_ORDER")) {
            uint32_t* d_bad = nullptr;
            if (hipMalloc(&d_bad, 8 * sizeof(uint32_t)) == hipSuccess) {
                for (int round = 0; round < 2; ++round) {
                    (void)hipMemsetAsync(d_bad, 0, 8 * sizeof(uint32_t), stream);
                    hipLaunchKernelGGL(k_check_order, dim3((n32 + 255) / 256), dim3(256), 0, stream, order, n32, d_bad);
                    uint32_t bad[8] = {};
                    (void)hipMemcpyAsync(bad, d_bad, sizeof(bad), hipMemcpyDeviceToHost, stream);
                    (void)hipStreamSynchronize(stream);
                    if (bad[0]) {
                        std::vector<uint32_t> host(n32);
                        (void)hipMemcpy(host.data(), order, size_t{n32} * 4, hipMemcpyDeviceToHost);
// ... 284 lines not shown
```

bvh_amd/csrc/upload.hip:

```cpp
#include "common.h"

#include <mutex>

namespace bvh_amd {

namespace {

template <typename T>
__global__ void __launch_bounds__(256) relayout_pairs(const HostNode<T>* nodes, size_t pair_count, PairNode<T>* out) {
    size_t p = blockIdx.x * size_t{256} + threadIdx.x;
    if (p >= pair_count) return;
    const HostNode<T>& l = nodes[2 * p + 1];
    const HostNode<T>& r = nodes[2 * p + 2];
    PairNode<T> rec;
#pragma unroll
    for (int k = 0; k < 6; ++k) { rec.lb[k] = l.bounds[k]; rec.rb[k] = r.bounds[k]; }
    rec.li = static_cast<uint32_t>(l.index);
    rec.ri = static_cast<uint32_t>(r.index);
#pragma unroll
    for (size_t k = 0; k < sizeof(rec.pad) / 4; ++k) rec.pad[k] = 0;
    out[p] = rec;
}

template <typename T>
__global__ void __launch_bounds__(256) k_depth_init(const PairNode<T>* pairs, uint32_t n_pairs, uint32_t root_pair, uint32_t* anc, uint32_t* dist) {
    const uint32_t p = blockIdx.x * 256 + threadIdx.x;
    if (p >= n_pairs) return;
    const uint32_t li = pairs[p].li, ri = pairs[p].ri;
    const uint32_t lp = li >> (kCountBits + 1), rp = ri >> (kCountBits + 1);
    if ((li & kCountMask) == 0 && lp < n_pairs && lp != root_pair) { anc[lp] = p; dist[lp] = 1; }
    if ((ri & kCountMask) == 0 && rp < n_pairs && rp != root_pair) { anc[rp] = p; dist[rp] = 1; }
}
__global__ void __launch_bounds__(256) k_depth_identity(uint32_t n, uint32_t* anc, uint32_t* dist) {
    const uint32_t i = blockIdx.x * 256 + threadIdx.x;
    if (i < n) { anc[i] = i; dist[i] = 0; }
}
__global__ void __launch_bounds__(256) k_depth_jump(const uint32_t* anc, const uint32_t* dist, uint32_t n, uint32_t* anc_out, uint32_t* dist_out,
                                                    uint32_t* max_out, uint32_t root_pair) {
    const uint32_t i = blockIdx.x * 256 + threadIdx.x;
    if (i >= n) return;
    const uint32_t a = anc[i], d = dist[i] + dist[a], top = anc[a];
    anc_out[i] = top;
    dist_out[i] = d;
    if (max_out && top == root_pair) atomicMax(max_out, d);
    if (max_out && anc[top] != top) atomicOr(max_out + 1, 1u);
}

template <typename T>
__global__ void __launch_bounds__(256) k_expected_visits(const PairNode<T>* pairs, uint32_t n_pairs, double inv_root_area, unsigned long long* sum) {
    const uint32_t p = blockIdx.x * 256 + threadIdx.x;
    unsigned long long mine = 0;
    if (p < n_pairs) {
        const PairNode<T>& q = pairs[p];
        auto share = [&](const T* b, uint32_t index) -> unsigned long long {
            if ((index & kCountMask) != 0) return 0;
            const double x = double(b[1]) - double(b[0]), y = double(b[3]) - double(b[2]), z = double(b[5]) - double(b[4]);
            const double r = (x * y + y * z + z * x) * inv_root_area;
            return r > 0 ? static_cast<unsigned long long>(fmin(r, 1.0) * 65536.0) : 0;
        };
        mine = share(q.lb, q.li) + share(q.rb, q.ri);
    }
    __shared__ unsigned long long part[4];
    for (int off = 32; off > 0; off >>= 1) mine += __shfl_down(mine, off);
    if ((threadIdx.x & 63) == 0) part[threadIdx.x >> 6] = mine;
    __syncthreads();
    if (threadIdx.x == 0) atomicAdd(sum, part[0] + part[1] + part[2] + part[3]);
}

}

template <typename T>
int tree_depth(const BvhImpl<T>& b, hipStream_t stream) {
    if (b.max_depth.load() >= 0) return BVH_AMD_OK;
    static std::mutex once;
    std::lock_guard<std::mutex> lock(once);
    if (b.max_depth.load() >= 0) return BVH_AMD_OK;
    if (b.pair_count == 0) { b.max_depth = 0; return BVH_AMD_OK; }
    if (const int rc = b.wait_refit()) return rc;
    const uint32_t n = static_cast<uint32_t>(b.pair_count);
    StreamScope scratch_on(stream);
    ScratchTag buf_tag;
    uint32_t* buf = nullptr;
    BVH_HIP_TRY(scratch_alloc(reinterpret_cast<void**>(&buf), (size_t{4} * n + 4) * sizeof(uint32_t), &buf_tag), BVH_AMD_ERR_HIP);
    uint32_t *anc = buf, *dist = buf + n, *anc2 = buf + 2 * size_t{n}, *dist2 = buf + 3 * size_t{n};
    uint32_t* d_max = buf + 4 * size_t{n};
    unsigned long long* d_visits = reinterpret_cast<unsigned long long*>(d_max + 2);
    hipError_t e = hipMemsetAsync(d_max, 0, 16, stream);
    const unsigned grid = (n + 255) / 256;
    {
        const double x = double(b.root_bounds[1]) - double(b.root_bounds[0]), y = double(b.root_bounds[3]) - double(b.root_bounds[2]),
                     z = b.dim == 3 ? double(b.root_bounds[5]) - double(b.root_bounds[4]) : 0.0;
        const double area = x * y + y * z + z * x;
        hipLaunchKernelGGL(k_expected_visits<T>, dim3(grid), dim3(256), 0, stream, b.d_pairs, n, area > 0 ? 1.0 / area : 0.0, d_visits);
    }
    hipLaunchKernelGGL(k_depth_identity, dim3(grid), dim3(256), 0, stream, n, anc, dist);
    hipLaunchKernelGGL(k_depth_init<T>, dim3(grid), dim3(256), 0, stream, b.d_pairs, n, b.root_index >> (kCountBits + 1), anc, dist);
    int rounds = 1;
    while ((uint64_t{1} << rounds) < uint64_t{n} + 1) ++rounds;
    uint32_t words[4] = {0, 0, 0, 0};
    int done = 0;
    for (const int upto : {std::min(rounds, 7), rounds}) {
        if (done >= upto) break;
        if (done) e = hipMemsetAsync(d_max, 0, 8, stream);
        for (int r = done; r < upto; ++r) {
            hipLaunchKernelGGL(k_depth_jump, dim3(grid), dim3(256), 0, stream, anc, dist, n, anc2, dist2, r == upto - 1 ? d_max : nullptr,
                               b.root_index >> (kCountBits + 1));
            std::swap(anc, anc2); std::swap(dist, dist2);
        }
        done = upto;
        if (e == hipSuccess) e = hipGetLastError();
        if (e == hipSuccess) e = hipMemcpyAsync(words, d_max, 16, hipMemcpyDeviceToHost, stream);
        if (e == hipSuccess) e = hipStreamSynchronize(stream);
        if (e != hipSuccess || words[1] == 0) break;
    }
    scratch_free(buf, buf_tag);
    if (e != hipSuccess) return fail(BVH_AMD_ERR_HIP, std::string("tree_depth: ") + hipGetErrorString(e));
    const uint32_t deepest = words[0];
    b.expected_visits = static_cast<float>(static_cast<double>((static_cast<unsigned long long>(words[3]) << 32) | words[2]) / 65536.0);
    b.max_depth = static_cast<int>(deepest) + 1;
    return BVH_AMD_OK;
}
template int tree_depth<float>(const BvhImpl<float>&, hipStream_t);
template int tree_depth<double>(const BvhImpl<double>&, hipStream_t);

template <typename T>
BvhImpl<T>::~BvhImpl() {
    if (device >= 0) {
        int cur = -1;
        (void)hipGetDevice(&cur);
        if (cur != device) (void)hipSetDevice(device);
        if (d_pairs) { scratch_forget(d_pairs); (void)hipFree(d_pairs); }
        if (d_prim_ids) { scratch_forget(d_prim_ids); (void)hipFree(d_prim_ids); }
        if (d_work) (void)hipFree(d_work);
        for (hipEvent_t& e : work_done) if (e) { (void)hipEventDestroy(e); e = nullptr; }
        for (PlanSearch& ps : plan_search) { if (ps.start) (void)hipEventDestroy(ps.start); if (ps.stop) (void)hipEventDestroy(ps.stop); ps.start = ps.stop = nullptr; }
        if (d_nodes) { scratch_forget(d_nodes); (void)hipFree(d_nodes); }
        if (refit_done) { (void)hipEventSynchronize(refit_done); (void)hipEventDestroy(refit_done); }
        if (h_root) (void)hipHostFree(h_root);
        if (cur >= 0 && cur != device) (void)hipSetDevice(cur);
    }
}

template <typename T>
int BvhImpl<T>::wait_refit() const {
    if (!root_pending.load(std::memory_order_acquire)) return BVH_AMD_OK;
    std::lock_guard<std::mutex> lock(root_mutex);
    if (!root_pending.load(std::memory_order_acquire)) return BVH_AMD_OK;
    BVH_HIP_TRY(hipEventSynchronize(refit_done), BVH_AMD_ERR_HIP);
    for (int k = 0; k < 6; ++k) root_bounds[k] = h_root->bounds[k];
    root_pending.store(false, std::memory_order_release);
    return BVH_AMD_OK;
}

template <typename T>
int BvhImpl<T>::note_refit(hipStream_t stream) {
    std::lock_guard<std::mutex> lock(root_mutex);
    if (!h_root) BVH_HIP_TRY(hipHostMalloc(reinterpret_cast<void**>(&h_root), sizeof(HostNode<T>), hipHostMallocDefault), BVH_AMD_ERR_HIP);
    if (!refit_done) BVH_HIP_TRY(hipEventCreateWithFlags(&refit_done, hipEventDisableTiming), BVH_AMD_ERR_HIP);
    BVH_HIP_TRY(hipMemcpyAsync(h_root, d_nodes, sizeof(HostNode<T>), hipMemcpyDeviceToHost, stream), BVH_AMD_ERR_HIP);
    BVH_HIP_TRY(hipEventRecord(refit_done, stream), BVH_AMD_ERR_HIP);
    root_pending.store(true, std::memory_order_release);
    return BVH_AMD_OK;
}

template <typename T>
int traversal_cost(const BvhImpl<T>& b, double* cost_out, hipStream_t stream) {
    int rc = b.wait_refit();
    if (rc) return rc;
    double cost = 0.0;
    if (b.pair_count) {
        StreamScope scratch_on(stream);
        ScratchTag tag;
        unsigned long long* d_sum = nullptr;
        BVH_HIP_TRY(scratch_alloc(reinterpret_cast<void**>(&d_sum), 16, &tag), BVH_AMD_ERR_HIP);
        const uint32_t n = static_cast<uint32_t>(b.pair_count);
        const double x = double(b.root_bounds[1]) - double(b.root_bounds[0]), y = double(b.root_bounds[3]) - double(b.root_bounds[2]),
                     z = double(b.root_bounds[5]) - double(b.root_bounds[4]);
        const double area = x * y + y * z + z * x;
        unsigned long long sum = 0;
        hipError_t e = hipMemsetAsync(d_sum, 0, 8, stream);
        hipLaunchKernelGGL(k_expected_visits<T>, dim3((n + 255) / 256), dim3(256), 0, stream, b.d_pairs, n, area > 0 ? 1.0 / area : 0.0, d_sum);
        if (e == hipSuccess) e = hipGetLastError();
        if (e == hipSuccess) e = hipMemcpyAsync(&sum, d_sum, 8, hipMemcpyDeviceToHost, stream);
        if (e == hipSuccess) e = hipStreamSynchronize(stream);
        scratch_free(d_sum, tag);
        if (e != hipSuccess) return fail(BVH_AMD_ERR_HIP, std::string("traversal_cost: ") + hipGetErrorString(e));
        cost = static_cast<double>(sum) / 65536.0;
    }
    b.expected_visits = static_cast<float>(cost);
    *cost_out = cost;
    return BVH_AMD_OK;
}
template int traversal_cost<float>(const BvhImpl<float>&, double*, hipStream_t);
template int traversal_cost<double>(const BvhImpl<double>&, double*, hipStream_t);

template <typename T>
int BvhImpl<T>::sync_host() const {
    if (host_valid.load(std::memory_order_acquire)) return BVH_AMD_OK;
    if (const int rc = wait_refit()) return rc;
    std::lock_guard<std::mutex> lock(host_mutex);
    if (host_valid.load(std::memory_order_acquire)) return BVH_AMD_OK;
    int cur = -1;
    BVH_HIP_TRY(hipGetDevice(&cur), BVH_AMD_ERR_HIP);
    if (cur != device) BVH_HIP_TRY(hipSetDevice(device), BVH_AMD_ERR_HIP);
    nodes.resize(node_count);
    std::vector<uint32_t> ids(prim_count);
    hipError_t e = hipMemcpy(nodes.data(), d_nodes, node_count * sizeof(HostNode<T>), hipMemcpyDeviceToHost);
    if (e == hipSuccess) e = hipMemcpy(ids.data(), d_prim_ids, prim_count * sizeof(uint32_t), hipMemcpyDeviceToHost);
    if (cur != device) (void)hipSetDevice(cur);
    if (e != hipSuccess) return fail(BVH_AMD_ERR_HIP, std::string("sync_host: ") + hipGetErrorString(e));
    prim_ids.assign(ids.begin(), ids.end());
    nodes2_valid.store(false);
    host_valid.store(true, std::memory_order_release);
    return BVH_AMD_OK;
}

template <typename T>
int relayout_on_device(BvhImpl<T>& b, const HostNode<T>* d_nodes, hipStream_t stream) {
    b.pair_count = (b.node_count - 1) / 2;
    b.max_depth = -1;
    b.max_prim_id = -1;
    { std::lock_guard<std::mutex> lock(b.plan_mutex); for (int k = 0; k < 2; ++k) { b.launch_plan[k] = 0; b.plan_search[k].index = 0; b.plan_search[k].pending = false; b.plan_search[k].trying = -1; b.plan_search[k].dropped = 0; for (auto& c : b.plan_search[k].count) c = 0; for (auto& t : b.plan_search[k].ns_per_ray) t = 0.0f; for (auto& r : b.plan_search[k].rays_of) r = 0; } }
    if (b.d_pairs) { scratch_forget(b.d_pairs); (void)hipFree(b.d_pairs); b.d_pairs = nullptr; }
    if (b.pair_count) {
        StreamScope scratch_on(stream);
        ScratchTag tag;
        BVH_HIP_TRY(scratch_alloc(reinterpret_cast<void**>(&b.d_pairs), b.pair_count * sizeof(PairNode<T>), &tag), BVH_AMD_ERR_HIP);
        unsigned grid = static_cast<unsigned>((b.pair_count + 255) / 256);
        hipLaunchKernelGGL(relayout_pairs<T>, dim3(grid), dim3(256), 0, stream, d_nodes, b.pair_count, b.d_pairs);
        BVH_HIP_TRY(hipGetLastError(), BVH_AMD_ERR_HIP);
    }
    return BVH_AMD_OK;
}

template <typename T>
int BvhImpl<T>::sync_host2() const {
    int rc = sync_host();
    if (rc) return rc;
    if (nodes2_valid.load(std::memory_order_acquire)) return BVH_AMD_OK;
    std::lock_guard<std::mutex> lock(host_mutex);
    if (!nodes2_valid.load(std::memory_order_acquire)) {
        nodes2.resize(nodes.size());
        for (size_t i = 0; i < nodes.size(); ++i) {
            for (int k = 0; k < 4; ++k) nodes2[i].bounds[k] = nodes[i].bounds[k];
            nodes2[i].index = nodes[i].index;
        }
        nodes2_valid.store(true, std::memory_order_release);
    }
    return BVH_AMD_OK;
}

template <typename T>
void BvhImpl<T>::widen_host() const {
    nodes.resize(nodes2.size());
    for (size_t i = 0; i < nodes2.size(); ++i) {
        for (int k = 0; k < 4; ++k) nodes[i].bounds[k] = nodes2[i].bounds[k];
        nodes[i].bounds[4] = nodes[i].bounds[5] = T(0);
        nodes[i].index = nodes2[i].index;
    }
}

template <typename T>
int upload_bvh(BvhImpl<T>& b, hipStream_t stream) {
    if (b.nodes.empty()) return fail(BVH_AMD_ERR_ARG, "upload: empty BVH");
    b.node_count = b.nodes.size(); b.prim_count = b.prim_ids.size(); b.host_valid = true;
    for (int k = 0; k < 6; ++k) b.root_bounds[k] = b.nodes[0].bounds[k];
    if (b.nodes.size() % 2 == 0) return fail(BVH_AMD_ERR_ARG, "upload: node count must be odd (root + sibling pairs)");
    if (b.nodes.size() >= (size_t{1} << 28) || b.prim_ids.size() >= (size_t{1} << 28))
        return fail(BVH_AMD_ERR_UNSUPPORTED, "upload: more than 2^28 nodes/primitives (32-bit device indices)");
    BVH_HIP_TRY(hipGetDevice(&b.device), BVH_AMD_ERR_HIP);
    if (!b.d_work) BVH_HIP_TRY(hipMalloc(&b.d_work, size_t{BvhImpl<T>::kWorkSlots} * BvhImpl<T>::kWorkStride * sizeof(unsigned long long)), BVH_AMD_ERR_HIP);
    b.root_index = static_cast<uint32_t>(b.nodes[0].index);

    HostNode<T>* d_nodes = nullptr;
    BVH_HIP_TRY(hipMalloc(&d_nodes, b.nodes.size() * sizeof(HostNode<T>)), BVH_AMD_ERR_HIP);
    hipError_t e = hipMemcpyAsync(d_nodes, b.nodes.data(), b.nodes.size() * sizeof(HostNode<T>), hipMemcpyHostToDevice, stream);
    int rc = e == hipSuccess ? validate_resident_nodes<T>(d_nodes, b.nodes.size(), b.prim_ids.size(), stream, "upload") : fail(BVH_AMD_ERR_HIP, hipGetErrorString(e));
    if (rc == BVH_AMD_OK) rc = relayout_on_device(b, d_nodes, stream);
    if (rc == BVH_AMD_OK) {
        std::vector<uint32_t> ids(b.prim_ids.size());
        for (size_t i = 0; i < ids.size(); ++i) ids[i] = static_cast<uint32_t>(b.prim_ids[i]);
        if (b.d_prim_ids) { (void)hipFree(b.d_prim_ids); b.d_prim_ids = nullptr; }
        e = hipMalloc(&b.d_prim_ids, std::max<size_t>(ids.size(), 1) * sizeof(uint32_t));
        if (e == hipSuccess) e = hipMemcpyAsync(b.d_prim_ids, ids.data(), ids.size() * sizeof(uint32_t), hipMemcpyHostToDevice, stream);
        if (e == hipSuccess) e = hipStreamSynchronize(stream);
        if (e != hipSuccess) rc = fail(BVH_AMD_ERR_HIP, hipGetErrorString(e));
    }
    (void)hipStreamSynchronize(stream);
    (void)hipFree(d_nodes);
    return rc;
}

template struct BvhImpl<float>;
template struct BvhImpl<double>;
template int upload_bvh<float>(BvhImpl<float>&, hipStream_t);
template int upload_bvh<double>(BvhImpl<double>&, hipStream_t);
template int relayout_on_device<float>(BvhImpl<float>&, const HostNode<float>*, hipStream_t);
template int relayout_on_device<double>(BvhImpl<double>&, const HostNode<double>*, hipStream_t);

}
```

include/bvh_amd.h:

```cpp
#ifndef BVH_AMD_H
#define BVH_AMD_H

#include <stddef.h>
#include <stdint.h>
#include <stdio.h>
#include <stdbool.h>

#ifdef __cplusplus
extern "C" {
#endif

#define BVH_AMD_API __attribute__((visibility("default")))

#define BVH_ROOT_INDEX 0
#define BVH_INVALID_PRIM_ID SIZE_MAX

struct bvh3f;
struct bvh3d;
struct bvh_node3f;
struct bvh_node3d;
struct bvh2f;
struct bvh2d;
struct bvh_node2f;
struct bvh_node2d;
// ... 186 lines not shown
BVH_AMD_API void bvh3d_append_node(struct bvh3d*);
BVH_AMD_API void bvh3f_remove_last_node(struct bvh3f*);
BVH_AMD_API void bvh3d_remove_last_node(struct bvh3d*);
BVH_AMD_API void bvh_node3f_set_prim_count(struct bvh_node3f*, size_t);
BVH_AMD_API void bvh_node3d_set_prim_count(struct bvh_node3d*, size_t);
BVH_AMD_API void bvh_node3f_set_first_id(struct bvh_node3f*, size_t);
BVH_AMD_API void bvh_node3d_set_first_id(struct bvh_node3d*, size_t);
BVH_AMD_API void bvh_node3f_set_bbox(struct bvh_node3f*, const struct bvh_bbox3f*);
BVH_AMD_API void bvh_node3d_set_bbox(struct bvh_node3d*, const struct bvh_bbox3d*);

BVH_AMD_API void bvh3f_save(const struct bvh3f*, FILE*);
BVH_AMD_API void bvh3d_save(const struct bvh3d*, FILE*);
BVH_AMD_API struct bvh3f* bvh3f_load(FILE*);
BVH_AMD_API struct bvh3d* bvh3d_load(FILE*);
BVH_AMD_API size_t bvh3f_serialize(const struct bvh3f*, void* out, size_t cap);
BVH_AMD_API size_t bvh3d_serialize(const struct bvh3d*, void* out, size_t cap);
BVH_AMD_API struct bvh3f* bvh3f_deserialize(const void* bytes, size_t size);
BVH_AMD_API struct bvh3d* bvh3d_deserialize(const void* bytes, size_t size);
BVH_AMD_API size_t bvh3f_serialize_device(struct bvh3f*, void* d_out, size_t cap, void* stream);
BVH_AMD_API size_t bvh3d_serialize_device(struct bvh3d*, void* d_out, size_t cap, void* stream);
BVH_AMD_API struct bvh3f* bvh3f_deserialize_device(const void* d_bytes, size_t size, void* stream);
BVH_AMD_API struct bvh3d* bvh3d_deserialize_device(const void* d_bytes, size_t size, void* stream);

BVH_AMD_API struct bvh_node3f* bvh3f_get_node(struct bvh3f*, size_t);
BVH_AMD_API struct bvh_node3d* bvh3d_get_node(struct bvh3d*, size_t);
BVH_AMD_API size_t bvh3f_get_prim_id(const struct bvh3f*, size_t);
BVH_AMD_API size_t bvh3d_get_prim_id(const struct bvh3d*, size_t);
BVH_AMD_API size_t bvh3f_get_prim_count(const struct bvh3f*);
BVH_AMD_API size_t bvh3d_get_prim_count(const struct bvh3d*);
BVH_AMD_API size_t bvh3f_get_node_count(const struct bvh3f*);
BVH_AMD_API size_t bvh3d_get_node_count(const struct bvh3d*);
BVH_AMD_API bool bvh_node3f_is_leaf(const struct bvh_node3f*);
BVH_AMD_API bool bvh_node3d_is_leaf(const struct bvh_node3d*);
BVH_AMD_API size_t bvh_node3f_get_prim_count(const struct bvh_node3f*);
BVH_AMD_API size_t bvh_node3d_get_prim_count(const struct bvh_node3d*);
BVH_AMD_API size_t bvh_node3f_get_first_id(const struct bvh_node3f*);
BVH_AMD_API size_t bvh_node3d_get_first_id(const struct bvh_node3d*);
BVH_AMD_API struct bvh_bbox3f bvh_node3f_get_bbox(const struct bvh_node3f*);
BVH_AMD_API struct bvh_bbox3d bvh_node3d_get_bbox(const struct bvh_node3d*);
BVH_AMD_API void bvh3f_copy_nodes(const struct bvh3f*, void* out_nodes28);
BVH_AMD_API void bvh3d_copy_nodes(const struct bvh3d*, void* out_nodes56);
BVH_AMD_API void bvh3f_copy_prim_ids(const struct bvh3f*, size_t* out);
BVH_AMD_API void bvh3d_copy_prim_ids(const struct bvh3d*, size_t* out);
BVH_AMD_API const uint32_t* bvh3f_device_prim_ids(const struct bvh3f*);
BVH_AMD_API const uint32_t* bvh3d_device_prim_ids(const struct bvh3d*);

BVH_AMD_API int bvh_amd_tri_bounds3f(const float* d_tris9, size_t n, float* d_bboxes, float* d_centers, void* stream);
BVH_AMD_API int bvh_amd_tri_bounds3d(const double* d_tris9, size_t n, double* d_bboxes, double* d_centers, void* stream);
BVH_AMD_API int bvh_amd_precompute_tris3f(const float* d_tris9, const uint32_t* d_perm, size_t n, float* d_tris12, void* stream);
BVH_AMD_API int bvh_amd_precompute_tris3d(const double* d_tris9, const uint32_t* d_perm, size_t n, double* d_tris12, void* stream);
BVH_AMD_API int bvh_amd_sphere_bounds3f(const float* d_sph4, size_t n, float* d_bboxes, float* d_centers, void* stream);
BVH_AMD_API int bvh_amd_sphere_bounds3d(const double* d_sph4, size_t n, double* d_bboxes, double* d_centers, void* stream);
BVH_AMD_API int bvh_amd_gather(const void* d_in, const uint32_t* d_perm, size_t n, size_t stride, void* d_out, void* stream);

BVH_AMD_API int bvh_amd_pinhole_rays3f(const float eye[3], const float dir[3], const float up[3], size_t width, size_t height,
    struct bvh_ray3f* d_rays, void* stream);
BVH_AMD_API int bvh_amd_pinhole_rays3d(const double eye[3], const double dir[3], const double up[3], size_t width, size_t height,
    struct bvh_ray3d* d_rays, void* stream);
BVH_AMD_API int bvh_amd_shade_eyelight3f(const float* d_tris12, const struct bvh_ray3f* d_rays, const struct bvh_hit3f* d_hits, size_t n,
    uint8_t* d_rgb, void* stream);
BVH_AMD_API int bvh_amd_shade_eyelight3d(const double* d_tris12, const struct bvh_ray3d* d_rays, const struct bvh_hit3d* d_hits, size_t n,
    uint8_t* d_rgb, void* stream);

BVH_AMD_API int bvh3f_intersect_rays_tri(const struct bvh3f*, const float* d_tris12, const struct bvh_ray3f* d_rays,
    size_t n, unsigned flags, struct bvh_hit3f* d_hits, struct bvh_amd_counters* d_counters, void* stream);
BVH_AMD_API int bvh3d_intersect_rays_tri(const struct bvh3d*, const double* d_tris12, const struct bvh_ray3d* d_rays,
    size_t n, unsigned flags, struct bvh_hit3d* d_hits, struct bvh_amd_counters* d_counters, void* stream);
BVH_AMD_API int bvh3f_intersect_rays_sphere(const struct bvh3f*, const float* d_sph4, const struct bvh_ray3f* d_rays,
    size_t n, unsigned flags, struct bvh_hit3f* d_hits, struct bvh_amd_counters* d_counters, void* stream);
BVH_AMD_API int bvh3d_intersect_rays_sphere(const struct bvh3d*, const double* d_sph4, const struct bvh_ray3d* d_rays,
    size_t n, unsigned flags, struct bvh_hit3d* d_hits, struct bvh_amd_counters* d_counters, void* stream);

BVH_AMD_API int bvh3f_closest_points_tri(const struct bvh3f*, const float* d_tris12, const float* d_queries4, size_t n, unsigned flags,
    struct bvh_hit3f* d_out, struct bvh_amd_counters* d_counters, void* stream);
BVH_AMD_API int bvh3d_closest_points_tri(const struct bvh3d*, const double* d_tris12, const double* d_queries4, size_t n, unsigned flags,
    struct bvh_hit3d* d_out, struct bvh_amd_counters* d_counters, void* stream);
BVH_AMD_API int bvh3f_closest_points_sphere(const struct bvh3f*, const float* d_sph4, const float* d_queries4, size_t n, unsigned flags,
    struct bvh_hit3f* d_out, struct bvh_amd_counters* d_counters, void* stream);
BVH_AMD_API int bvh3d_closest_points_sphere(const struct bvh3d*, const double* d_sph4, const double* d_queries4, size_t n, unsigned flags,
    struct bvh_hit3d* d_out, struct bvh_amd_counters* d_counters, void* stream);

BVH_AMD_API int bvh3f_prepare_trace(const struct bvh3f*, size_t n_rays_hint, void* stream);
BVH_AMD_API int bvh3d_prepare_trace(const struct bvh3d*, size_t n_rays_hint, void* stream);

BVH_AMD_API int bvh_amd_std_sort_ids3f(const float* d_keys, size_t n, uint32_t* d_ids_out, void* stream);
BVH_AMD_API int bvh_amd_std_sort_ids3d(const double* d_keys, size_t n, uint32_t* d_ids_out, void* stream);
BVH_AMD_API int bvh_amd_radix_sort_pairs_u32(uint32_t* d_keys, uint32_t* d_vals, size_t n, int bits, void* stream);

BVH_AMD_API const char* bvh_amd_last_kernel_name(void);
BVH_AMD_API int bvh_amd_last_launch_reordered(void);
BVH_AMD_API void bvh_amd_kernel_timing(int on);
BVH_AMD_API int bvh_amd_kernel_times(float* ms_out, size_t capacity, size_t* count_out);
BVH_AMD_API int bvh_amd_reorder_times(float* ms_out, size_t capacity, size_t* count_out);
BVH_AMD_API void bvh_amd_tuning(int refill_threshold, int leaf_threshold, int coop_fetch, int ticket_ranges);
BVH_AMD_API int bvh_amd_experiment(const char* name, int value);
BVH_AMD_API int bvh_amd_wave_times(unsigned long long* out, size_t capacity_waves, size_t* n_waves);
BVH_AMD_API void bvh_amd_last_launch_plan(int out[4]);
BVH_AMD_API void bvh_amd_last_plan_search(float ns_per_ray[5], int measurements[5], unsigned* dropped_mask);
BVH_AMD_API void bvh_amd_reinsertion_stats(unsigned out[2]);
struct bvh_amd_optimize_profile { unsigned iterations, replayed; unsigned long long replacements; float heap_ms; };
BVH_AMD_API void bvh_amd_last_optimize_profile(struct bvh_amd_optimize_profile* out);


BVH_AMD_API void bvh3f_intersect_ray(const struct bvh3f*, const struct bvh_ray3f*, const struct bvh_intersect_callbackf*);
BVH_AMD_API void bvh3d_intersect_ray(const struct bvh3d*, const struct bvh_ray3d*, const struct bvh_intersect_callbackd*);
BVH_AMD_API void bvh3f_intersect_ray_any(const struct bvh3f*, const struct bvh_ray3f*, const struct bvh_intersect_callbackf*);
BVH_AMD_API void bvh3d_intersect_ray_any(const struct bvh3d*, const struct bvh_ray3d*, const struct bvh_intersect_callbackd*);
BVH_AMD_API void bvh3f_intersect_ray_robust(const struct bvh3f*, const struct bvh_ray3f*, const struct bvh_intersect_callbackf*);
BVH_AMD_API void bvh3d_intersect_ray_robust(const struct bvh3d*, const struct bvh_ray3d*, const struct bvh_intersect_callbackd*);
BVH_AMD_API void bvh3f_intersect_ray_any_robust(const struct bvh3f*, const struct bvh_ray3f*, const struct bvh_intersect_callbackf*);
BVH_AMD_API void bvh3d_intersect_ray_any_robust(const struct bvh3d*, const struct bvh_ray3d*, const struct bvh_intersect_callbackd*);
#define BVH_AMD_START_AT_ROOT SIZE_MAX
BVH_AMD_API int bvh3f_intersect_ray_visit(const struct bvh3f*, const struct bvh_ray3f*, size_t start_index, unsigned flags,
    const struct bvh_amd_ray_visitorf*);
BVH_AMD_API int bvh3d_intersect_ray_visit(const struct bvh3d*, const struct bvh_ray3d*, size_t start_index, unsigned flags,
    const struct bvh_amd_ray_visitord*);

BVH_AMD_API struct bvh2f* bvh2f_build(struct bvh_thread_pool*, const struct bvh_bbox2f* bboxes,
    const struct bvh_vec2f* centers, size_t prim_count, const struct bvh_build_config* config);
BVH_AMD_API struct bvh2f* bvh2f_build_device(const float* d_bboxes4, const float* d_centers2, size_t prim_count,
    const struct bvh_build_config* config, enum bvh_amd_builder builder, void* stream);
BVH_AMD_API struct bvh2f* bvh2f_build_sah(struct bvh_thread_pool*, const struct bvh_bbox2f* bboxes, const struct bvh_vec2f* centers,
    size_t prim_count, const struct bvh_build_config* config, const struct bvh_amd_sah_config* sah);
BVH_AMD_API struct bvh2f* bvh2f_build_device_sah(const float* d_bboxes4, const float* d_centers2, size_t prim_count,
    const struct bvh_build_config* config, enum bvh_amd_builder builder, const struct bvh_amd_sah_config* sah, void* stream);
BVH_AMD_API struct bvh2f* bvh2f_build_device_binned(const float* d_bboxes4, const float* d_centers2, size_t prim_count,
    const struct bvh_build_config* config, const struct bvh_amd_sah_config* sah, size_t bin_count, void* stream);
BVH_AMD_API struct bvh2f* bvh2f_from_nodes(const void* nodes, size_t node_count, const size_t* prim_ids, size_t prim_count);
BVH_AMD_API struct bvh2f* bvh2f_extract(struct bvh2f* bvh, size_t root_id);
BVH_AMD_API void bvh2f_destroy(struct bvh2f*);
BVH_AMD_API void bvh2f_optimize(struct bvh_thread_pool*, struct bvh2f*);
BVH_AMD_API int bvh2f_optimize_config(struct bvh2f*, const struct bvh_amd_optimize_config*);
BVH_AMD_API void bvh2f_refit(struct bvh2f*);
BVH_AMD_API int bvh2f_refit_status(struct bvh2f*);
BVH_AMD_API int bvh2f_refit_boxes(struct bvh2f*, const float* d_bboxes4, size_t n_boxes, void* stream);
BVH_AMD_API int bvh2f_sync_device(struct bvh2f*);
BVH_AMD_API void bvh2f_append_node(struct bvh2f*);
BVH_AMD_API void bvh2f_remove_last_node(struct bvh2f*);
BVH_AMD_API void bvh_node2f_set_prim_count(struct bvh_node2f*, size_t);
BVH_AMD_API void bvh_node2f_set_first_id(struct bvh_node2f*, size_t);
BVH_AMD_API void bvh_node2f_set_bbox(struct bvh_node2f*, const struct bvh_bbox2f*);
BVH_AMD_API void bvh2f_save(const struct bvh2f*, FILE*);
BVH_AMD_API struct bvh2f* bvh2f_load(FILE*);
BVH_AMD_API size_t bvh2f_serialize(const struct bvh2f*, void* out, size_t capacity);
BVH_AMD_API struct bvh2f* bvh2f_deserialize(const void* bytes, size_t size);
BVH_AMD_API size_t bvh2f_serialize_device(struct bvh2f*, void* d_out, size_t cap, void* stream);
BVH_AMD_API struct bvh2f* bvh2f_deserialize_device(const void* d_bytes, size_t size, void* stream);
BVH_AMD_API struct bvh_node2f* bvh2f_get_node(struct bvh2f*, size_t);
BVH_AMD_API size_t bvh2f_get_prim_id(const struct bvh2f*, size_t);
BVH_AMD_API size_t bvh2f_get_prim_count(const struct bvh2f*);
BVH_AMD_API size_t bvh2f_get_node_count(const struct bvh2f*);
BVH_AMD_API bool bvh_node2f_is_leaf(const struct bvh_node2f*);
BVH_AMD_API size_t bvh_node2f_get_prim_count(const struct bvh_node2f*);
BVH_AMD_API size_t bvh_node2f_get_first_id(const struct bvh_node2f*);
BVH_AMD_API struct bvh_bbox2f bvh_node2f_get_bbox(const struct bvh_node2f*);
BVH_AMD_API void bvh2f_copy_nodes(const struct bvh2f*, void* out);
BVH_AMD_API void bvh2f_copy_prim_ids(const struct bvh2f*, size_t* out);
BVH_AMD_API const uint32_t* bvh2f_device_prim_ids(const struct bvh2f*);
BVH_AMD_API int bvh_amd_sphere_bounds2f(const float* d_circles3, size_t n, float* d_bboxes4, float* d_centers2, void* stream);
BVH_AMD_API int bvh2f_intersect_rays_sphere(const struct bvh2f* bvh, const float* d_circles3, const struct bvh_ray2f* d_rays,
    size_t n, unsigned flags, struct bvh_hit3f* d_hits, struct bvh_amd_counters* d_counters, void* stream);

BVH_AMD_API struct bvh2d* bvh2d_build(struct bvh_thread_pool*, const struct bvh_bbox2d* bboxes,
    const struct bvh_vec2d* centers, size_t prim_count, const struct bvh_build_config* config);
BVH_AMD_API struct bvh2d* bvh2d_build_device(const double* d_bboxes4, const double* d_centers2, size_t prim_count,
    const struct bvh_build_config* config, enum bvh_amd_builder builder, void* stream);
// ... 68 lines not shown
```

Measured before the change: 2415 Mrays/s.

## Cull stale traversal stack entries using stored 16-bit entry distances

Closest-hit traversal kernels now store a truncated 16-bit entry distance in LDS for the first stack levels. When an entry is popped whose distance already exceeds the current tmax, its node-pair fetch and box tests are skipped. This is only safe when child boxes nest inside their parents, so a one-time device check now runs alongside the depth computation and is cached. In exchange, the LDS stack shrinks from 20 to 16 entries in these kernels, which can cause more spills, and each push and pop does extra LDS traffic. The lane-prefix popcount is also replaced with the mbcnt intrinsic.

```diff
diff --git a/bvh_amd/_lib.py b/bvh_amd/_lib.py
--- a/bvh_amd/_lib.py
+++ b/bvh_amd/_lib.py
@@ -143,6 +143,7 @@
     "bvh{S}_intersect_rays_tri": (_I, [_P, _P, _P, _Z, _U, _P, _P, _P]),
     "bvh{S}_intersect_rays_sphere": (_I, [_P, _P, _P, _Z, _U, _P, _P, _P]),
     "bvh{S}_prepare_trace": (_I, [_P, _Z, _P]),
+    "bvh{S}_boxes_nested": (_I, [_P, C.POINTER(C.c_int), _P]),
     "bvh{S}_closest_points_tri": (_I, [_P, _P, _P, _Z, _U, _P, _P, _P]),
     "bvh{S}_closest_points_sphere": (_I, [_P, _P, _P, _Z, _U, _P, _P, _P]),
     "bvh{S}_intersect_ray": (None, [_P, _P, _P]),
@@ -175,7 +176,7 @@
     return Visitor, leaf_t, inner_t
 
 
-_ONLY_3D = ("bvh_amd_tri_bounds{S}", "bvh_amd_precompute_tris{S}", "bvh{S}_intersect_rays_tri", "bvh{S}_prepare_trace",
+_ONLY_3D = ("bvh_amd_tri_bounds{S}", "bvh_amd_precompute_tris{S}", "bvh{S}_intersect_rays_tri", "bvh{S}_prepare_trace", "bvh{S}_boxes_nested",
             "bvh{S}_build_minitree_device",
             "bvh{S}_closest_points_tri", "bvh{S}_closest_points_sphere",
             "bvh{S}_refit_tris", "bvh{S}_traversal_cost")
diff --git a/bvh_amd/api.py b/bvh_amd/api.py
--- a/bvh_amd/api.py
+++ b/bvh_amd/api.py
@@ -200,6 +200,14 @@
         cost = C.c_double(0.0)
         _lib.check(self._f("bvh{S}_traversal_cost")(self._h, C.byref(cost), _stream()), "traversal_cost")
         return float(cost.value)
+
+    def boxes_nested(self) -> bool:
+        _torch()
+        if self.dim != 3:
+            raise TypeError("boxes_nested: 3D trees only")
+        out = C.c_int(0)
+        _lib.check(self._f("bvh{S}_boxes_nested")(self._h, C.byref(out), _stream()), "boxes_nested")
+        return bool(out.value)
 
     def set_node_bbox(self, node_id: int, lo, hi):
         node = self._f("bvh{S}_get_node")(self._h, node_id)
diff --git a/bvh_amd/csrc/capi.hip b/bvh_amd/csrc/capi.hip
--- a/bvh_amd/csrc/capi.hip
+++ b/bvh_amd/csrc/capi.hip
@@ -327,6 +327,7 @@
     }
     rc = refit_prims_device<T>(b.d_nodes, b.d_pairs, b.node_count, src_kind, d_src, n_src, b.d_prim_ids, b.prim_count, stream);
     if (rc == BVH_AMD_OK && d_tris12_out) rc = launch_precompute_tris<T>(d_src, b.d_prim_ids, b.prim_count, d_tris12_out, stream);
+    b.nested = -1;
     b.host_valid = false;
     b.nodes2_valid = false;
     const int rc2 = b.note_refit(stream);
@@ -727,7 +728,16 @@
         int cur = -1;                                                                                               \
         BVH_HIP_TRY(hipGetDevice(&cur), BVH_AMD_ERR_HIP);                                                           \
         if (cur != impl<T>(b)->device) return fail(BVH_AMD_ERR_ARG, "prepare_trace: BVH lives on another device than the current one"); \
-        return prepare_trace<T>(*impl<T>(b), n_rays_hint, static_cast<hipStream_t>(s)); }
+        return prepare_trace<T>(*impl<T>(b), n_rays_hint, static_cast<hipStream_t>(s)); }                           \
+    int bvh##S##_boxes_nested(const bvh##S* b, int* nested_out, void* s) {                                         \
+        if (!b || !nested_out) return fail(BVH_AMD_ERR_ARG, "boxes_nested: null bvh or output");                    \
+        int cur = -1;                                                                                               \
+        BVH_HIP_TRY(hipGetDevice(&cur), BVH_AMD_ERR_HIP);                                                           \
+        if (cur != impl<T>(b)->device) return fail(BVH_AMD_ERR_ARG, "boxes_nested: BVH lives on another device than the current one"); \
+        if (impl<T>(b)->pair_count && !impl<T>(b)->d_pairs) return fail(BVH_AMD_ERR_ARG, "boxes_nested: BVH has no device nodes"); \
+        const int rc = boxes_nested<T>(*impl<T>(b), static_cast<hipStream_t>(s));                                  \
+        if (rc == BVH_AMD_OK) *nested_out = impl<T>(b)->nested.load() == 1 ? 1 : 0;                                 \
+        return rc; }
 
 BVH_AMD_IMPL(float, 3f)
 BVH_AMD_IMPL(double, 3d)
diff --git a/bvh_amd/csrc/common.h b/bvh_amd/csrc/common.h
--- a/bvh_amd/csrc/common.h
+++ b/bvh_amd/csrc/common.h
@@ -107,6 +107,7 @@
     uint32_t root_index = 0;
     mutable std::atomic<int> max_depth{-1};
     mutable std::atomic<float> expected_visits{0.0f};
+    mutable std::atomic<int> nested{-1};
     mutable std::atomic<uint32_t> launch_plan[2] = {};
     struct PlanSearch {
         int index = 0;
@@ -180,6 +181,7 @@
 
 template <typename T> int upload_bvh(BvhImpl<T>& b, hipStream_t stream);
 template <typename T> int tree_depth(const BvhImpl<T>& b, hipStream_t stream);
+template <typename T> int boxes_nested(const BvhImpl<T>& b, hipStream_t stream);
 template <typename T> int prepare_trace(const BvhImpl<T>& b, size_t n_rays_hint, hipStream_t stream);
 
 template <typename T> int relayout_on_device(BvhImpl<T>& b, const HostNode<T>* d_nodes, hipStream_t stream);
diff --git a/bvh_amd/csrc/trace_body.inc b/bvh_amd/csrc/trace_body.inc
--- a/bvh_amd/csrc/trace_body.inc
+++ b/bvh_amd/csrc/trace_body.inc
@@ -1,13 +1,18 @@
 #ifndef BVH_TRACE_COOP
 #define BVH_TRACE_COOP false
 #endif
-    constexpr int kDepth = kLdsDepth;
+#ifndef BVH_TRACE_CULL
+#define BVH_TRACE_CULL false
+#endif
+    constexpr bool Cull = BVH_TRACE_CULL && !Any && !Stats && sizeof(T) == 4;
+    constexpr int kDepth = Cull ? kCullLdsDepth : kLdsDepth;
     constexpr int kSpill = 64 - kDepth;
     __shared__ uint32_t lds_stack[kDepth * kBlock];
+    __shared__ uint16_t lds_dist[Cull ? kCullLevels * kBlock : 1];
+    const uint32_t cull_levels = Cull ? min(a.cull, static_cast<uint32_t>(kCullLevels)) : 0u;
     uint32_t spill[kSpill];
     const int tid = threadIdx.x;
     const int lane = tid & (kWave - 1);
-    const uint64_t lanes_below = (uint64_t{1} << lane) - 1;
 
     bool have = false, done = false, drained = false, nan_ray = false;
     uint32_t part = a.parts > 1 ? blockIdx.x % a.parts : 0, parts_left = a.parts;
@@ -25,7 +30,8 @@
 #endif
 
     auto deep_slot = [&](uint32_t i) { return a.deep + (size_t{blockIdx.x} * kBlock + tid) * a.deep_cap + i; };
-    auto push = [&](uint32_t v) {
+    auto push = [&](uint32_t v, T entry) {
+        if constexpr (Cull) { if (sp < kCullLevels) lds_dist[sp * kBlock + tid] = entry_dist16(entry); }
         if (sp < kDepth) lds_stack[sp * kBlock + tid] = v;
         else if (!Deep) spill[min(sp - kDepth, static_cast<uint32_t>(kSpill - 1))] = v;
         else if (sp < kDepth + kSpill) spill[sp - kDepth] = v;
@@ -42,6 +48,21 @@
         }
         return v;
     };
+    auto pop_culled = [&]() -> uint32_t {
+        uint32_t s = 0;
+        if constexpr (Cull) s = lds_half(&lds_dist[min(sp - 1, static_cast<uint32_t>(kCullLevels - 1)) * kBlock + tid]);
+        uint32_t v = pop();
+        if constexpr (Cull) {
+            const bool drop = ((v & kCountMask) == 0) & (sp < cull_levels) & ((s << 16) > __float_as_uint(tmax));
+            if (drop) {
+                v = kCulledTop;
+#if defined(BVH_TRACE_CULL_PROBE)
+                BVH_TRACE_CULL_PROBE;
+#endif
+            }
+        }
+        return v;
+    };
 
     for (;;) {
         const uint64_t idle = __ballot(!have);
@@ -67,7 +88,7 @@
                 }
             }
             if (!have) {
-                const unsigned long long ticket = base + __popcll(idle & lanes_below);
+                const unsigned long long ticket = base + count_lanes_below(idle, lane);
                 if (ticket < part_end) {
                     const bool once = (a.stream_hints & 1u) != 0;
                     const unsigned long long my = a.order ? (once ? load_word_nt(a.order + ticket) : a.order[ticket]) : ticket;
@@ -118,9 +139,10 @@
             if (parked >= a.leaf_threshold) break;
             T lb[6], rb[6];
             uint32_t li = 0, ri = 0;
-            if constexpr (BVH_TRACE_COOP) coop_load_pair(a.pairs, a.pair_bytes, inner ? (top >> (kCountBits + 1)) : 0xFFFFFFFFu, lane, lb, rb, li, ri);
+            const bool culled = Cull && top == kCulledTop;
+            if constexpr (BVH_TRACE_COOP) coop_load_pair(a.pairs, a.pair_bytes, inner && !culled ? (top >> (kCountBits + 1)) : 0xFFFFFFFFu, lane, lb, rb, li, ri);
             if (inner) {
-                if constexpr (!BVH_TRACE_COOP) load_pair(a.pairs + (top >> (kCountBits + 1)), lb, rb, li, ri);
+                if constexpr (!BVH_TRACE_COOP) { if (!culled) load_pair(a.pairs + (top >> (kCountBits + 1)), lb, rb, li, ri); }
                 if (Stats) ++n_pairs;
                 T l0 = tmin, l1 = tmax, r0 = tmin, r1 = tmax;
 #pragma unroll
@@ -138,13 +160,15 @@
                     l0 = Num<T>::max_num(la, l0); l1 = Num<T>::min_num(lz, l1);
                     r0 = Num<T>::max_num(ra, r0); r1 = Num<T>::min_num(rz, r1);
                 }
-                const bool hl = !nan_ray && l0 <= l1, hr = !nan_ray && r0 <= r1;
+                const bool live = !nan_ray && !culled;
+                const bool hl = live && l0 <= l1, hr = live && r0 <= r1;
                 if (hl) {
                     uint32_t near_i = li;
                     if (hr) {
                         uint32_t far_i = ri;
-                        if (!Any && l0 > r0) { near_i = ri; far_i = li; }
-                        push(far_i);
+                        T far_t = r0;
+                        if (!Any && l0 > r0) { near_i = ri; far_i = li; far_t = l0; }
+                        push(far_i, far_t);
                     }
                     top = near_i;
                 } else if (hr) {
@@ -152,7 +176,7 @@
                 } else if (sp == 0) {
                     done = true;
                 } else {
-                    top = pop();
+                    top = pop_culled();
                 }
             }
         }
@@ -204,7 +228,7 @@
             }
             if (Any && hit_prim != BVH_AMD_INVALID) done = true;
             else if (sp == 0) done = true;
-            else top = pop();
+            else top = pop_culled();
         }
 
         if (have && done) {
diff --git a/bvh_amd/csrc/trace_device.h b/bvh_amd/csrc/trace_device.h
--- a/bvh_amd/csrc/trace_device.h
+++ b/bvh_amd/csrc/trace_device.h
@@ -12,6 +12,8 @@
 
 constexpr int kBlock = 256;
 constexpr int kLdsDepth = 20;
+constexpr int kCullLdsDepth = 16, kCullLevels = 8;
+constexpr uint32_t kCulledTop = 0xFFFFFFFFu << (kCountBits + 1);
 constexpr int kRefillThreshold = 36;
 constexpr int kRefillThresholdSmall = 20;
 constexpr int kLeafThreshold = 12;
@@ -62,6 +64,27 @@
 #endif
 }
 
+__device__ inline int count_lanes_below(uint64_t mask, int lane) {
+#if defined(__HIP_DEVICE_COMPILE__)
+    (void)lane;
+    return static_cast<int>(__builtin_amdgcn_mbcnt_hi(static_cast<uint32_t>(mask >> 32), __builtin_amdgcn_mbcnt_lo(static_cast<uint32_t>(mask), 0u)));
+#else
+    return __builtin_popcountll(mask & ((uint64_t{1} << lane) - 1));
+#endif
+}
+__device__ inline uint32_t lds_half(const uint16_t* shared) {
+#if defined(__HIP_DEVICE_COMPILE__)
+    typedef __attribute__((address_space(3))) const volatile uint16_t LdsHalf;
+    return *(LdsHalf*)shared;
+#else
+    return *shared;
+#endif
+}
+__device__ inline uint16_t entry_dist16(float t) {
+    const uint32_t bits = __float_as_uint(t);
+    return static_cast<uint16_t>(bits - 1u < 0x7F7FFFFFu ? bits >> 16 : 0u);
+}
+
 template <typename T> __device__ inline T dot2(T a0, T a1, T b0, T b1) { return (T(0) + a0 * b0) + a1 * b1; }
 
 constexpr uint32_t kTicketStride = 16;
@@ -90,6 +113,7 @@
     uint32_t one_shot;
     unsigned long long* wave_times;
     uint32_t pair_bytes = 0;
+    uint32_t cull = 0;
 };
 
 __device__ inline void load_pair(const PairNode<float>* p, float (&lb)[6], float (&rb)[6], uint32_t& li, uint32_t& ri) {
@@ -222,6 +246,24 @@
 }
 #endif
 
+template <typename T>
+__device__ inline bool record_nested(const PairNode<T>* pairs, uint32_t n_pairs, uint32_t p) {
+    const PairNode<T>& q = pairs[p];
+    bool ok = true;
+    for (int k = 0; k < 6; ++k)
+        ok = ok && q.lb[k] >= -Num<T>::kMax && q.lb[k] <= Num<T>::kMax && q.rb[k] >= -Num<T>::kMax && q.rb[k] <= Num<T>::kMax;
+    auto inside = [&](const T* outer, uint32_t index) {
+        const uint32_t c = index >> (kCountBits + 1);
+        if ((index & kCountMask) != 0 || c >= n_pairs) return true;
+        const PairNode<T>& r = pairs[c];
+        bool in = true;
+        for (int k = 0; k < 3; ++k)
+            in = in && r.lb[2 * k] >= outer[2 * k] && r.lb[2 * k + 1] <= outer[2 * k + 1] && r.rb[2 * k] >= outer[2 * k] && r.rb[2 * k + 1] <= outer[2 * k + 1];
+        return in;
+    };
+    return ok && inside(q.lb, q.li) && inside(q.rb, q.ri);
+}
+
 __device__ inline void load_prim12(const float* p, float (&v)[12]) {
     const float4* q = reinterpret_cast<const float4*>(p);
     float4 a = q[0], b = q[1], c = q[2];
diff --git a/bvh_amd/csrc/traverse.hip b/bvh_amd/csrc/traverse.hip
--- a/bvh_amd/csrc/traverse.hip
+++ b/bvh_amd/csrc/traverse.hip
@@ -42,7 +42,10 @@
     constexpr bool Deep = false;
 #undef BVH_TRACE_COOP
 #define BVH_TRACE_COOP true
+#undef BVH_TRACE_CULL
+#define BVH_TRACE_CULL true
 #include "trace_body.inc"
+#undef BVH_TRACE_CULL
 #undef BVH_TRACE_COOP
 }
 
@@ -67,7 +70,10 @@
     constexpr bool Deep = false, Stats = false;
 #undef BVH_TRACE_COOP
 #define BVH_TRACE_COOP true
+#undef BVH_TRACE_CULL
+#define BVH_TRACE_CULL true
 #include "trace_body.inc"
+#undef BVH_TRACE_CULL
 #undef BVH_TRACE_COOP
 }
 
@@ -145,7 +151,7 @@
 
 thread_local int t_refill = -1, t_leaf = -1, t_coop = -1, t_parts = -1;
 struct Experiments { int grid_blocks = -1, stream_hints = -1, tri_stride = -1, key_curve = -1, key_bits = -1, step_events = -1, wave_times = -1, one_shot = -1,
-                     key_class_bits = -1, key_class_scale = -1, stagger = -1; };
+                     key_class_bits = -1, key_class_scale = -1, stagger = -1, cull = -1; };
 constexpr int kKeyClassBits = 0, kKeyClassScalePercent = 500;
 constexpr uint32_t kStaggerHeavy = 100000, kStaggerLight = 50000, kStaggerDouble = 20000;
 thread_local bool g_last_classes = false;
@@ -460,6 +466,7 @@
     else if (k == "stagger") t_exp.stagger = value;
     else if (k == "key_class_bits") t_exp.key_class_bits = value;
     else if (k == "key_class_scale") t_exp.key_class_scale = value;
+    else if (k == "cull") t_exp.cull = value;
     else if (k == "wave_times") {
 #if defined(BVH_AMD_DEVELOPER)
         t_exp.wave_times = value;
@@ -633,6 +640,11 @@
         const int leaf_default = !args.coop ? kLeafThreshold : any_hit ? kCoopLeafAny : heavy ? kCoopLeafHeavy : kCoopLeafAny;
         args.refill_threshold = t_refill > 0 ? t_refill : refill_env > 0 ? refill_env : refill_default;
         args.leaf_threshold = t_leaf > 0 ? t_leaf : leaf_env > 0 ? leaf_env : leaf_default;
+    }
+    args.cull = 0;
+    if (args.coop && !any_hit && !d_counters && !args.deep && std::is_same_v<T, float> && b.dim == 3 && t_exp.cull != 0) {
+        if (const int rc = boxes_nested<T>(b, stream)) return release(rc);
+        if (b.nested.load() == 1) args.cull = static_cast<uint32_t>(kCullLevels);
     }
     auto zero_tickets = [&]() -> int {
         const hipError_t e = hipMemsetAsync(work, 0, size_t{args.parts} * kTicketStride * sizeof(unsigned long long), stream);
diff --git a/bvh_amd/csrc/upload.hip b/bvh_amd/csrc/upload.hip
--- a/bvh_amd/csrc/upload.hip
+++ b/bvh_amd/csrc/upload.hip
@@ -1,6 +1,8 @@
 #include "common.h"
+#include "trace_device.h"
 
 #include <mutex>
+#include <type_traits>
 
 namespace bvh_amd {
 
@@ -67,6 +69,12 @@
     if (threadIdx.x == 0) atomicAdd(sum, part[0] + part[1] + part[2] + part[3]);
 }
 
+template <typename T>
+__global__ void __launch_bounds__(256) k_boxes_nested(const PairNode<T>* pairs, uint32_t n_pairs, uint32_t* not_nested) {
+    const uint32_t p = blockIdx.x * 256 + threadIdx.x;
+    if (p < n_pairs && !record_nested(pairs, n_pairs, p)) atomicOr(not_nested, 1u);
+}
+
 }
 
 template <typename T>
@@ -75,18 +83,19 @@
     static std::mutex once;
     std::lock_guard<std::mutex> lock(once);
     if (b.max_depth.load() >= 0) return BVH_AMD_OK;
-    if (b.pair_count == 0) { b.max_depth = 0; return BVH_AMD_OK; }
+    if (b.pair_count == 0) { b.nested = 1; b.max_depth = 0; return BVH_AMD_OK; }
     if (const int rc = b.wait_refit()) return rc;
     const uint32_t n = static_cast<uint32_t>(b.pair_count);
     StreamScope scratch_on(stream);
     ScratchTag buf_tag;
     uint32_t* buf = nullptr;
-    BVH_HIP_TRY(scratch_alloc(reinterpret_cast<void**>(&buf), (size_t{4} * n + 4) * sizeof(uint32_t), &buf_tag), BVH_AMD_ERR_HIP);
+    BVH_HIP_TRY(scratch_alloc(reinterpret_cast<void**>(&buf), (size_t{4} * n + 8) * sizeof(uint32_t), &buf_tag), BVH_AMD_ERR_HIP);
     uint32_t *anc = buf, *dist = buf + n, *anc2 = buf + 2 * size_t{n}, *dist2 = buf + 3 * size_t{n};
     uint32_t* d_max = buf + 4 * size_t{n};
     unsigned long long* d_visits = reinterpret_cast<unsigned long long*>(d_max + 2);
-    hipError_t e = hipMemsetAsync(d_max, 0, 16, stream);
+    hipError_t e = hipMemsetAsync(d_max, 0, 20, stream);
     const unsigned grid = (n + 255) / 256;
+    hipLaunchKernelGGL(k_boxes_nested<T>, dim3(grid), dim3(256), 0, stream, b.d_pairs, n, d_max + 4);
     {
         const double x = double(b.root_bounds[1]) - double(b.root_bounds[0]), y = double(b.root_bounds[3]) - double(b.root_bounds[2]),
                      z = b.dim == 3 ? double(b.root_bounds[5]) - double(b.root_bounds[4]) : 0.0;
@@ -97,7 +106,7 @@
     hipLaunchKernelGGL(k_depth_init<T>, dim3(grid), dim3(256), 0, stream, b.d_pairs, n, b.root_index >> (kCountBits + 1), anc, dist);
     int rounds = 1;
     while ((uint64_t{1} << rounds) < uint64_t{n} + 1) ++rounds;
-    uint32_t words[4] = {0, 0, 0, 0};
+    uint32_t words[5] = {0, 0, 0, 0, 0};
     int done = 0;
     for (const int upto : {std::min(rounds, 7), rounds}) {
         if (done >= upto) break;
@@ -109,7 +118,7 @@
         }
         done = upto;
         if (e == hipSuccess) e = hipGetLastError();
-        if (e == hipSuccess) e = hipMemcpyAsync(words, d_max, 16, hipMemcpyDeviceToHost, stream);
+        if (e == hipSuccess) e = hipMemcpyAsync(words, d_max, 20, hipMemcpyDeviceToHost, stream);
         if (e == hipSuccess) e = hipStreamSynchronize(stream);
         if (e != hipSuccess || words[1] == 0) break;
     }
@@ -117,11 +126,35 @@
     if (e != hipSuccess) return fail(BVH_AMD_ERR_HIP, std::string("tree_depth: ") + hipGetErrorString(e));
     const uint32_t deepest = words[0];
     b.expected_visits = static_cast<float>(static_cast<double>((static_cast<unsigned long long>(words[3]) << 32) | words[2]) / 65536.0);
+    b.nested = words[4] ? 0 : 1;
     b.max_depth = static_cast<int>(deepest) + 1;
     return BVH_AMD_OK;
 }
 template int tree_depth<float>(const BvhImpl<float>&, hipStream_t);
 template int tree_depth<double>(const BvhImpl<double>&, hipStream_t);
+
+template <typename T>
+int boxes_nested(const BvhImpl<T>& b, hipStream_t stream) {
+    if (b.nested.load() >= 0) return BVH_AMD_OK;
+    if (b.max_depth.load() < 0) return tree_depth<T>(b, stream);
+    if (b.pair_count == 0) { b.nested = 1; return BVH_AMD_OK; }
+    StreamScope scratch_on(stream);
+    ScratchTag tag;
+    uint32_t* d_flag = nullptr;
+    BVH_HIP_TRY(scratch_alloc(reinterpret_cast<void**>(&d_flag), 16, &tag), BVH_AMD_ERR_HIP);
+    const uint32_t n = static_cast<uint32_t>(b.pair_count);
+    uint32_t flag = 0;
+    hipError_t e = hipMemsetAsync(d_flag, 0, 4, stream);
+    hipLaunchKernelGGL(k_boxes_nested<T>, dim3((n + 255) / 256), dim3(256), 0, stream, b.d_pairs, n, d_flag);
+    if (e == hipSuccess) e = hipGetLastError();
+    int rc = e == hipSuccess ? readback(&flag, d_flag, 4, stream) : fail(BVH_AMD_ERR_HIP, std::string("boxes_nested: ") + hipGetErrorString(e));
+    scratch_free(d_flag, tag);
+    if (rc) return rc;
+    b.nested = flag ? 0 : 1;
+    return BVH_AMD_OK;
+}
+template int boxes_nested<float>(const BvhImpl<float>&, hipStream_t);
+template int boxes_nested<double>(const BvhImpl<double>&, hipStream_t);
 
 template <typename T>
 BvhImpl<T>::~BvhImpl() {
@@ -219,6 +252,7 @@
 int relayout_on_device(BvhImpl<T>& b, const HostNode<T>* d_nodes, hipStream_t stream) {
     b.pair_count = (b.node_count - 1) / 2;
     b.max_depth = -1;
+    b.nested = -1;
     b.max_prim_id = -1;
     { std::lock_guard<std::mutex> lock(b.plan_mutex); for (int k = 0; k < 2; ++k) { b.launch_plan[k] = 0; b.plan_search[k].index = 0; b.plan_search[k].pending = false; b.plan_search[k].trying = -1; b.plan_search[k].dropped = 0; for (auto& c : b.plan_search[k].count) c = 0; for (auto& t : b.plan_search[k].ns_per_ray) t = 0.0f; for (auto& r : b.plan_search[k].rays_of) r = 0; } }
     if (b.d_pairs) { scratch_forget(b.d_pairs); (void)hipFree(b.d_pairs); b.d_pairs = nullptr; }
diff --git a/include/bvh_amd.h b/include/bvh_amd.h
--- a/include/bvh_amd.h
+++ b/include/bvh_amd.h
@@ -292,6 +292,9 @@
 
 BVH_AMD_API int bvh3f_prepare_trace(const struct bvh3f*, size_t n_rays_hint, void* stream);
 BVH_AMD_API int bvh3d_prepare_trace(const struct bvh3d*, size_t n_rays_hint, void* stream);
+
+BVH_AMD_API int bvh3f_boxes_nested(const struct bvh3f*, int* nested_out, void* stream);
+BVH_AMD_API int bvh3d_boxes_nested(const struct bvh3d*, int* nested_out, void* stream);
 
 BVH_AMD_API int bvh_amd_std_sort_ids3f(const float* d_keys, size_t n, uint32_t* d_ids_out, void* stream);
 BVH_AMD_API int bvh_amd_std_sort_ids3d(const double* d_keys, size_t n, uint32_t* d_ids_out, void* stream);
```

After: 2376 Mrays/s. 1.6% lower.
